# EleutherAI/DALLE-mtf

Hardware: AMD Instinct MI355X
Metric: train tokens/sec (text+image) per node, dalle_example (higher is better)
Workload: dtype bf16

## Files before the change

### dalle-mtf_amd/csrc/elementwise.hip

```cpp
#include "common.h"
#include <stdarg.h>

static thread_local char g_err[512] = "ok";
void dmi_set_error(const char* fmt, ...) {
  va_list ap;
  va_start(ap, fmt);
  vsnprintf(g_err, sizeof(g_err), fmt, ap);
  va_end(ap);
}
extern "C" const char* dmi_last_error_string(void) { return g_err; }
extern "C" int dmi_version(void) { return 100; }

__global__ __launch_bounds__(256) void embed_fwd_kernel(const int* __restrict__ tokens,
                                                        const bf16_t* __restrict__ wte,
                                                        const bf16_t* __restrict__ wpe, bf16_t* __restrict__ x,
                                                        int64_t rows, int S, int d, int vocab, const int* __restrict__ pos_dev) {
  const int lane = threadIdx.x & 63, wid = threadIdx.x >> 6;
  const int64_t row = (int64_t)blockIdx.x * 4 + wid;
  if (row >= rows) return;
  int tok = tokens[row];
  tok = tok < 0 ? 0 : (tok >= vocab ? vocab - 1 : tok);
  int s = (int)(row % S);
  if (pos_dev) {
    s = *pos_dev;
// ... 145 lines not shown
    float acc[8] = {0, 0, 0, 0, 0, 0, 0, 0};
    int cur = first_tok;
    bool open = head_open;
    bool first = true;
    for (int64_t i = i0; i < i1; ++i) {
      const int t = sorted_tok[i];
      if (t != cur) {
        float* dst = open ? part + ((int64_t)chunk * 2 + 0) * d + c * 8 : dwte + (int64_t)eb_clamp(cur, vocab) * d + c * 8;
        *(f32x4*)dst = f32x4{acc[0], acc[1], acc[2], acc[3]};
        *(f32x4*)(dst + 4) = f32x4{acc[4], acc[5], acc[6], acc[7]};
#pragma unroll
        for (int j = 0; j < 8; ++j) acc[j] = 0.f;
        cur = t;
        open = false;
        first = false;
      }
      float f[8];
      unpack8(*(const u32x4*)(dx + (int64_t)perm[i] * d + c * 8), f);
#pragma unroll
      for (int j = 0; j < 8; ++j) acc[j] += f[j];
    }
    const bool tail_open = (i1 < n) && (sorted_tok[i1] == cur);
    float* dst;
    if (open || tail_open) dst = part + ((int64_t)chunk * 2 + (first ? 0 : 1)) * d + c * 8;
    else dst = dwte + (int64_t)eb_clamp(cur, vocab) * d + c * 8;
    *(f32x4*)dst = f32x4{acc[0], acc[1], acc[2], acc[3]};
    *(f32x4*)(dst + 4) = f32x4{acc[4], acc[5], acc[6], acc[7]};
  }
}
__global__ __launch_bounds__(256) void embed_bwd_wte_combine_kernel(const int* __restrict__ sorted_tok, float* __restrict__ dwte,
                                                                    const float* __restrict__ part, int64_t n, int d, int vocab) {
  const int lane = threadIdx.x & 63, wid = threadIdx.x >> 6;
  const int64_t chunk = (int64_t)blockIdx.x * 4 + wid;
  const int64_t i0 = chunk * EB_CH;
  if (i0 >= n) return;
  const int64_t i1 = (i0 + EB_CH < n) ? i0 + EB_CH : n;
  if (i1 >= n) return;
  const int tok = sorted_tok[i1 - 1];
  if (sorted_tok[i1] != tok) return;
  const bool single = sorted_tok[i0] == tok;
  if (single && i0 > 0 && sorted_tok[i0 - 1] == tok) return;
  const int slot = single ? 0 : 1;
  const int64_t nchunks = (n + EB_CH - 1) / EB_CH;
  int64_t cnt = 0;
  for (int64_t base = chunk + 1; base < nchunks; base += 64) {
    const int64_t k = base + lane;
    bool cont = false, last = true;
    if (k < nchunks) {
      const int64_t k0 = k * EB_CH, k1 = (k0 + EB_CH < n) ? k0 + EB_CH : n;
      cont = sorted_tok[k0] == tok;
      last = !(sorted_tok[k1 - 1] == tok && k1 < n && sorted_tok[k1] == tok);
    }
    const unsigned long long stop = __ballot(!cont || last);
    if (stop == 0ull) { cnt += 64; continue; }
    const int f = __ffsll((long long)stop) - 1;
    const unsigned long long contb = __ballot(cont);
    cnt += f + (((contb >> f) & 1ull) ? 1 : 0);
    break;
  }
  const float* p0 = part + ((int64_t)chunk * 2 + slot) * d;
  const float* pk = part + ((int64_t)(chunk + 1) * 2) * d;
  for (int c = lane; c < d / 4; c += 64) {
    f32x4 acc = *(const f32x4*)(p0 + c * 4);
    int64_t k = 0;
    for (; k + 4 <= cnt; k += 4) {
      const f32x4 v0 = *(const f32x4*)(pk + (k + 0) * 2 * d + c * 4);
      const f32x4 v1 = *(const f32x4*)(pk + (k + 1) * 2 * d + c * 4);
      const f32x4 v2 = *(const f32x4*)(pk + (k + 2) * 2 * d + c * 4);
      const f32x4 v3 = *(const f32x4*)(pk + (k + 3) * 2 * d + c * 4);
#pragma unroll
      for (int j = 0; j < 4; ++j) acc[j] = (((acc[j] + v0[j]) + v1[j]) + v2[j]) + v3[j];
    }
    for (; k < cnt; ++k) {
      const f32x4 v = *(const f32x4*)(pk + k * 2 * d + c * 4);
      acc[0] += v[0]; acc[1] += v[1]; acc[2] += v[2]; acc[3] += v[3];
    }
    *(f32x4*)(dwte + (int64_t)eb_clamp(tok, vocab) * d + c * 4) = acc;
  }
}

extern "C" int64_t dmi_embed_bwd_workspace_bytes(int B, int S, int d) {
  return (((int64_t)B * S + EB_CH - 1) / EB_CH) * 2 * d * 4 + 256;
}
extern "C" int dmi_embed_bwd(const int32_t* sorted_tokens, const int32_t* perm, const uint16_t* dx, float* dwte,
                             float* dwpe, int B, int S, int d, int vocab, void* workspace, void* stream) {
  DMI_REQUIRE(sorted_tokens && perm && dx && dwte && dwpe && workspace, "embed_bwd: null pointer");
  DMI_REQUIRE(d % 8 == 0 && B > 0 && S > 0 && vocab > 0, "embed_bwd: bad sizes");
  hipStream_t st = (hipStream_t)stream;
  embed_bwd_wpe_kernel<<<dim3((S + 3) / 4), dim3(256), 0, st>>>(dx, dwpe, B, S, d);
  DMI_CHECK_LAUNCH("embed_bwd_wpe");
  DMI_REQUIRE(hipMemsetAsync(dwte, 0, (size_t)vocab * d * 4, st) == hipSuccess, "embed_bwd: memset failed");
  const int64_t n = (int64_t)B * S;
  const int64_t chunks = cdiv64(n, EB_CH);
  embed_bwd_wte_sorted_kernel<<<dim3((unsigned)cdiv64(chunks, 4)), dim3(256), 0, st>>>(sorted_tokens, perm, dx, dwte, (float*)workspace, n, d, vocab);
  DMI_CHECK_LAUNCH("embed_bwd_wte_sorted");
  embed_bwd_wte_combine_kernel<<<dim3((unsigned)cdiv64(chunks, 4)), dim3(256), 0, st>>>(sorted_tokens, dwte, (const float*)workspace, n, d, vocab);
  DMI_CHECK_LAUNCH("embed_bwd_wte_combine");
  return DMI_OK;
}

template <int NC>
__global__ __launch_bounds__(256) void ln_fwd_kernel(const bf16_t* __restrict__ x, const bf16_t* __restrict__ g,
                                                     const bf16_t* __restrict__ b, bf16_t* __restrict__ y,
                                                     float* __restrict__ mean, float* __restrict__ rstd,
                                                     int64_t rows, int d, float eps) {
  const int lane = threadIdx.x & 63, wid = threadIdx.x >> 6;
  const int64_t row = (int64_t)blockIdx.x * 4 + wid;
  if (row >= rows) return;
  const int nch = d / 8;
  float v[NC][8];
  float sum = 0.f;
#pragma unroll
  for (int i = 0; i < NC; ++i) {
    const int c = lane + 64 * i;
    if (c < nch) {
      unpack8(*(const u32x4*)(x + row * d + c * 8), v[i]);
#pragma unroll
      for (int j = 0; j < 8; ++j) sum += v[i][j];
    }
  }
  const float mu = wave_sum(sum) / (float)d;
  float sq = 0.f;
#pragma unroll
  for (int i = 0; i < NC; ++i) {
    const int c = lane + 64 * i;
    if (c < nch) {
#pragma unroll
      for (int j = 0; j < 8; ++j) {
        v[i][j] -= mu;
        sq += v[i][j] * v[i][j];
      }
    }
  }
  const float rs = rsqrtf(wave_sum(sq) / (float)d + eps);
#pragma unroll
  for (int i = 0; i < NC; ++i) {
    const int c = lane + 64 * i;
    if (c < nch) {
      float fg[8], fb[8], o[8];
      unpack8(*(const u32x4*)(g + c * 8), fg);
      unpack8(*(const u32x4*)(b + c * 8), fb);
#pragma unroll
      for (int j = 0; j < 8; ++j) o[j] = v[i][j] * rs * fg[j] + fb[j];
      *(u32x4*)(y + row * d + c * 8) = pack8(o);
    }
  }
  if (lane == 0) {
    mean[row] = mu;
    rstd[row] = rs;
  }
}

extern "C" int dmi_layernorm_fwd(const uint16_t* x, const uint16_t* g, const uint16_t* b, uint16_t* y, float* mean,
                                 float* rstd, int64_t rows, int d, float eps, void* stream) {
  DMI_REQUIRE(x && g && b && y && mean && rstd, "layernorm_fwd: null pointer");
  DMI_REQUIRE(d % 8 == 0 && d <= 4096 && rows > 0, "layernorm_fwd: unsupported d=%d (need d%%8==0, d<=4096)", d);
  hipStream_t st = (hipStream_t)stream;
  dim3 grid((unsigned)cdiv64(rows, 4)), blk(256);
  if (d <= 512) ln_fwd_kernel<1><<<grid, blk, 0, st>>>(x, g, b, y, mean, rstd, rows, d, eps);
  else if (d <= 1024) ln_fwd_kernel<2><<<grid, blk, 0, st>>>(x, g, b, y, mean, rstd, rows, d, eps);
  else if (d <= 2048) ln_fwd_kernel<4><<<grid, blk, 0, st>>>(x, g, b, y, mean, rstd, rows, d, eps);
  else ln_fwd_kernel<8><<<grid, blk, 0, st>>>(x, g, b, y, mean, rstd, rows, d, eps);
  DMI_CHECK_LAUNCH("layernorm_fwd");
  return DMI_OK;
}

__global__ __launch_bounds__(256) void reduce_partials_kernel(const float* __restrict__ part, float* __restrict__ out,
                                                              int P, int ncols) {
  __shared__ float sm[4][64];
  const int cl = threadIdx.x & 63, grp = threadIdx.x >> 6;
  const int c = blockIdx.x * 64 + cl;
  float acc = 0.f;
  if (c < ncols) {
    float a0 = 0.f, a1 = 0.f, a2 = 0.f, a3 = 0.f;
    int p = grp;
    for (; p + 12 < P; p += 16) {
      a0 += part[(int64_t)p * ncols + c];
      a1 += part[(int64_t)(p + 4) * ncols + c];
      a2 += part[(int64_t)(p + 8) * ncols + c];
      a3 += part[(int64_t)(p + 12) * ncols + c];
    }
    for (; p < P; p += 4) a0 += part[(int64_t)p * ncols + c];
    acc = (a0 + a1) + (a2 + a3);
  }
  sm[grp][cl] = acc;
  __syncthreads();
  if (grp == 0 && c < ncols) out[c] = (sm[0][cl] + sm[1][cl]) + (sm[2][cl] + sm[3][cl]);
}

#define LN_BWD_RPB 32
extern "C" int64_t dmi_layernorm_bwd_workspace_bytes(int64_t rows, int d) {
  return cdiv64(rows, LN_BWD_RPB) * 2 * (int64_t)d * 4;
}

template <int NC>
__global__ __launch_bounds__(256) void ln_bwd_kernel(const bf16_t* __restrict__ dy, const bf16_t* __restrict__ x,
                                                     const bf16_t* __restrict__ g, const float* __restrict__ mean,
                                                     const float* __restrict__ rstd, const bf16_t* __restrict__ dres,
                                                     bf16_t* __restrict__ dx, float* __restrict__ part,
                                                     int64_t rows, int d) {
  extern __shared__ __attribute__((aligned(16))) float sm[];
  const int lane = threadIdx.x & 63, wid = threadIdx.x >> 6;
  const int nch = d / 8;
  float ag[NC][8], ab[NC][8], fg[NC][8];
#pragma unroll
  for (int i = 0; i < NC; ++i) {
    const int c = lane + 64 * i;
#pragma unroll
    for (int j = 0; j < 8; ++j) ag[i][j] = ab[i][j] = 0.f;
    if (c < nch) unpack8(*(const u32x4*)(g + c * 8), fg[i]);
  }
  const int64_t r0 = (int64_t)blockIdx.x * LN_BWD_RPB;
  u32x4 rdy[NC], rx[NC], rr[NC];
  float mu_n = 0.f, rs_n = 0.f;
  auto fetch = [&](int64_t row) {
    if (row < rows) {
      mu_n = mean[row];
      rs_n = rstd[row];
#pragma unroll
      for (int i = 0; i < NC; ++i) {
        const int c = lane + 64 * i;
        if (c < nch) {
          rdy[i] = *(const u32x4*)(dy + row * d + c * 8);
          rx[i] = *(const u32x4*)(x + row * d + c * 8);
          if (dres) rr[i] = *(const u32x4*)(dres + row * d + c * 8);
        }
      }
    }
  };
  fetch(r0 + wid);
  for (int it = 0; it < LN_BWD_RPB / 4; ++it) {
    const int64_t row = r0 + wid + 4 * it;
    if (row >= rows) break;
    const float mu = mu_n, rs = rs_n;
    float fy[NC][8], xh[NC][8], fr[NC][8];
    float s1 = 0.f, s2 = 0.f;
#pragma unroll
    for (int i = 0; i < NC; ++i) {
      const int c = lane + 64 * i;
      if (c < nch) {
        float fx[8];
        unpack8(rdy[i], fy[i]);
        unpack8(rx[i], fx);
        if (dres) unpack8(rr[i], fr[i]);
#pragma unroll
        for (int j = 0; j < 8; ++j) {
// ... 123 lines not shown
  float a0 = 0.f, a1 = 0.f, a2 = 0.f, a3 = 0.f, a4 = 0.f, a5 = 0.f, a6 = 0.f, a7 = 0.f;
  if (c < nc) {
    int p = grp;
    for (; p + 112 < P; p += 128) {
      const float* q = part + (int64_t)p * nc + c;
      a0 += q[0];
      a1 += q[16 * nc];
      a2 += q[32 * nc];
      a3 += q[48 * nc];
      a4 += q[64 * nc];
      a5 += q[80 * nc];
      a6 += q[96 * nc];
      a7 += q[112 * nc];
    }
    for (; p < P; p += 16) a0 += part[(int64_t)p * nc + c];
  }
  sm[grp][cl] = ((a0 + a1) + (a2 + a3)) + ((a4 + a5) + (a6 + a7));
  __syncthreads();
  if (grp == 0 && c < nc) {
    float s = 0.f;
#pragma unroll
    for (int q = 0; q < 16; ++q) s += sm[q][cl];
    if (c < d) b.dg[it][c] = s;
    else b.db[it][c - d] = s;
  }
}
extern "C" int dmi_layernorm_bwd_finish_batch(const void* const* workspaces, float* const* dgs, float* const* dbs, const int64_t* rows,
                                              int n, int d, void* stream) {
  DMI_REQUIRE(workspaces && dgs && dbs && rows && n >= 1 && n <= LN_FINISH_MAX, "layernorm_bwd_finish_batch: 1..%d items", LN_FINISH_MAX);
  DMI_REQUIRE(d % 8 == 0 && d <= 2048, "layernorm_bwd_finish_batch: unsupported d=%d", d);
  LnFinishBatch b;
  b.d = d;
  for (int i = 0; i < n; ++i) {
    DMI_REQUIRE(workspaces[i] && dgs[i] && dbs[i] && rows[i] > 0, "layernorm_bwd_finish_batch: null pointer in item %d", i);
    b.part[i] = (const float*)workspaces[i]; b.dg[i] = dgs[i]; b.db[i] = dbs[i];
    b.P[i] = (int)cdiv64(rows[i], LN_BWD_RPB);
  }
  ln_bwd_finish_batch_kernel<<<dim3((2 * d + 15) / 16, n), dim3(256), 0, (hipStream_t)stream>>>(b);
  DMI_CHECK_LAUNCH("layernorm_bwd_finish_batch");
  return DMI_OK;
}

#define COLSUM_RPB 256
extern "C" int64_t dmi_colsum_workspace_bytes(int64_t M, int N) { return cdiv64(M, COLSUM_RPB) * (int64_t)N * 4; }

__global__ __launch_bounds__(256) void colsum_kernel(const bf16_t* __restrict__ Y, int ldy, float* __restrict__ part,
                                                     int64_t M, int N) {
  __shared__ float sm[4][64][8];
  const int cl = threadIdx.x & 63, rl = threadIdx.x >> 6;
  const int cg = blockIdx.x * 64 + cl;
  const int64_t r0 = (int64_t)blockIdx.y * COLSUM_RPB;
  const int64_t r1 = (r0 + COLSUM_RPB < M) ? r0 + COLSUM_RPB : M;
  float acc[8] = {0, 0, 0, 0, 0, 0, 0, 0};
  if (cg * 8 < N) {
    for (int64_t r = r0 + rl; r < r1; r += 4) {
      float f[8];
      unpack8(*(const u32x4*)(Y + r * ldy + cg * 8), f);
#pragma unroll
      for (int j = 0; j < 8; ++j) acc[j] += f[j];
    }
  }
#pragma unroll
  for (int j = 0; j < 8; ++j) sm[rl][cl][j] = acc[j];
  __syncthreads();
  if (rl == 0 && cg * 8 < N) {
#pragma unroll
    for (int j = 0; j < 8; ++j)
      part[(int64_t)blockIdx.y * N + cg * 8 + j] = (sm[0][cl][j] + sm[1][cl][j]) + (sm[2][cl][j] + sm[3][cl][j]);
  }
}

extern "C" int dmi_colsum(const uint16_t* Y, int ldy, float* out, int64_t M, int N, void* workspace, void* stream) {
  DMI_REQUIRE(Y && out && workspace, "colsum: null pointer");
  DMI_REQUIRE(N % 8 == 0 && ldy % 8 == 0 && M > 0, "colsum: N,ldy must be multiples of 8");
  hipStream_t st = (hipStream_t)stream;
  const int P = (int)cdiv64(M, COLSUM_RPB);
  colsum_kernel<<<dim3((N / 8 + 63) / 64, P), dim3(256), 0, st>>>(Y, ldy, (float*)workspace, M, N);
  DMI_CHECK_LAUNCH("colsum");
  reduce_partials_kernel<<<dim3((N + 63) / 64), dim3(256), 0, st>>>((const float*)workspace, out, P, N);
  DMI_CHECK_LAUNCH("colsum_reduce");
  return DMI_OK;
}

__device__ __forceinline__ void transpose_tile(const bf16_t* __restrict__ src, bf16_t* __restrict__ dst, int Rv, int R,
                                               int C, int64_t sr, int r0, int c0, unsigned (*t)[33]) {
  const int tid = threadIdx.x;
  {
    const int chunk = tid & 7, rp = tid >> 3;
    const int ra = r0 + 2 * rp, c = c0 + 8 * chunk;
    u32x4 va = {0, 0, 0, 0}, vb = {0, 0, 0, 0};
    if (c < C) {
      if (ra < Rv) va = *(const u32x4*)(src + (int64_t)ra * sr + c);
      if (ra + 1 < Rv) vb = *(const u32x4*)(src + (int64_t)(ra + 1) * sr + c);
    }
#pragma unroll
    for (int j = 0; j < 8; ++j) {
      const unsigned lo = (va[j >> 1] >> ((j & 1) * 16)) & 0xffffu;
      const unsigned hi = (vb[j >> 1] >> ((j & 1) * 16)) & 0xffffu;
      t[8 * chunk + j][rp] = lo | (hi << 16);
    }
  }
  __syncthreads();
  {
    const int orow = tid >> 2, seg = tid & 3;
    const int c = c0 + orow, r = r0 + 16 * seg;
    if (c < C) {
#pragma unroll
      for (int q = 0; q < 2; ++q) {
        const int rr = r + 8 * q;
        if (rr < R) {
          u32x4 v;
#pragma unroll
          for (int i = 0; i < 4; ++i) v[i] = t[orow][8 * seg + 4 * q + i];
          *(u32x4*)(dst + (int64_t)c * R + rr) = v;
        }
      }
    }
  }
}

__global__ __launch_bounds__(256) void transpose_kernel(const bf16_t* __restrict__ in, bf16_t* __restrict__ out,
                                                        int nh, int Rv, int R, int C, int64_t sb, int64_t sh, int64_t sr) {
  __shared__ unsigned t[64][33];
  const int bh = blockIdx.z, b = bh / nh, h = bh % nh;
  transpose_tile(in + b * sb + h * sh, out + (int64_t)bh * C * R, Rv, R, C, sr, blockIdx.y * 64, blockIdx.x * 64, t);
}

__global__ __launch_bounds__(256) void transpose_batch_kernel(const bf16_t* __restrict__ in, bf16_t* __restrict__ out,
                                                              const int64_t* __restrict__ table, int n) {
  __shared__ unsigned t[64][33];
  const int64_t tile = blockIdx.x;
  int i = 0;
  while (i + 1 < n && table[(i + 1) * 5 + 4] <= tile) ++i;
  const int64_t in_off = table[i * 5], out_off = table[i * 5 + 1];
  const int R = (int)table[i * 5 + 2], C = (int)table[i * 5 + 3];
  const int local = (int)(tile - table[i * 5 + 4]);
  const int tc = (C + 63) / 64;
  transpose_tile(in + in_off, out + out_off, R, R, C, C, (local / tc) * 64, (local % tc) * 64, t);
}
extern "C" int dmi_transpose_bf16_batch(const uint16_t* in_base, uint16_t* out_base, const int64_t* table, int n,
                                        int64_t total_tiles, void* stream) {
  DMI_REQUIRE(in_base && out_base && table && n > 0 && total_tiles > 0, "transpose_batch: bad args");
  transpose_batch_kernel<<<dim3((unsigned)total_tiles), dim3(256), 0, (hipStream_t)stream>>>(in_base, out_base, table, n);
  DMI_CHECK_LAUNCH("transpose_batch");
  return DMI_OK;
}

static int dmi_transpose_padded(const uint16_t* in, uint16_t* out, int nb, int nh, int Rv, int Rp, int C,
                         int64_t in_b_stride, int64_t in_h_stride, int64_t in_r_stride, void* stream) {
  DMI_REQUIRE(in && out, "transpose: null pointer");
  DMI_REQUIRE(Rp % 8 == 0 && Rp >= Rv && C % 8 == 0 && in_r_stride % 8 == 0 && in_h_stride % 8 == 0 && in_b_stride % 8 == 0,
              "transpose: R, C and strides must be multiples of 8 (R=%d C=%d)", Rp, C);
  transpose_kernel<<<dim3((C + 63) / 64, (Rp + 63) / 64, nb * nh), dim3(256), 0, (hipStream_t)stream>>>(
      in, out, nh, Rv, Rp, C, in_b_stride, in_h_stride, in_r_stride);
  DMI_CHECK_LAUNCH("transpose");
  return DMI_OK;
}
extern "C" int dmi_transpose_bf16_padded(const uint16_t* in, uint16_t* out, int R_valid, int R_pitch, int C, void* stream) {
  return dmi_transpose_padded(in, out, 1, 1, R_valid, R_pitch, C, 0, 0, C, stream);
}
extern "C" int dmi_transpose_bf16(const uint16_t* in, uint16_t* out, int batch, int R, int C, void* stream) {
  return dmi_transpose_padded(in, out, batch, 1, R, R, C, (int64_t)R * C, 0, C, stream);
}

__global__ void shift_labels_kernel(const int* __restrict__ tokens, int* __restrict__ labels, int B, int S, int eos) {
  const int64_t i = (int64_t)blockIdx.x * blockDim.x + threadIdx.x;
  if (i >= (int64_t)B * S) return;
  const int s = (int)(i % S);
  labels[i] = (s == S - 1) ? eos : tokens[i + 1];
}
extern "C" int dmi_shift_labels(const int32_t* tokens, int32_t* labels, int B, int S, int eos, void* stream) {
  DMI_REQUIRE(tokens && labels && B > 0 && S > 0, "shift_labels: bad args");
  const int64_t n = (int64_t)B * S;
  shift_labels_kernel<<<dim3((unsigned)cdiv64(n, 256)), dim3(256), 0, (hipStream_t)stream>>>(tokens, labels, B, S, eos);
  DMI_CHECK_LAUNCH("shift_labels");
  return DMI_OK;
}

__global__ __launch_bounds__(256) void assemble_tokens_kernel(const int* __restrict__ text,
                                                              const float* __restrict__ logits, int* __restrict__ out,
                                                              int B, int T, int P, int C, int text_vocab) {
  const int lane = threadIdx.x & 63, wid = threadIdx.x >> 6;
  const int64_t idx = (int64_t)blockIdx.x * 4 + wid;
  const int S = T + P;
  if (idx >= (int64_t)B * S) return;
  const int b = (int)(idx / S), s = (int)(idx % S);
  if (s < T) {
    if (lane == 0) out[idx] = text[(int64_t)b * T + s];
    return;
  }
  const float* row = logits + ((int64_t)b * P + (s - T)) * C;
  float best = -INFINITY;
  int bi = 0x7fffffff;
  for (int c = lane; c < C; c += 64) {
    const float v = row[c];
    if (v > best || (v == best && c < bi)) {
      best = v;
      bi = c;
    }
  }
#pragma unroll
// ... 143 lines not shown
  __syncthreads();
  const float k = dz_scale / bs;
  const int lch = (label >= 0 && label < V) ? (label >> 3) : -1, lj = label & 7;
#pragma unroll
  for (int i = 0; i < NC; ++i) {
    const int c = tid + 1024 * i;
    if (c < nch) {
#pragma unroll
      for (int j = 0; j < 8; ++j) f[i][j] *= k;
      if (c == lch) {
        asm volatile("" ::: "memory");
#pragma unroll
        for (int j = 0; j < 8; ++j) f[i][j] -= (j == lj) ? dz_scale : 0.f;
      }
      *(u32x4*)(zr + c * 8) = pack8(f[i]);
    }
  }
}

extern "C" int dmi_cross_entropy(uint16_t* z, int ldz, const int32_t* labels, float* loss_rows, float* lse,
                                 int64_t M, int V, float dz_scale, void* stream) {
  DMI_REQUIRE(z && labels && loss_rows, "cross_entropy: null pointer");
  DMI_REQUIRE(ldz % 8 == 0 && ldz >= ((V + 7) / 8) * 8 && M > 0 && V > 0, "cross_entropy: ldz must be a multiple of 8 and >= round_up(V,8)");
  hipStream_t st = (hipStream_t)stream;
  const int nch = ldz / 8;
  if (nch > 2048 && nch <= 8 * 1024) {
    if (nch <= 4 * 1024) cross_entropy_reg_kernel<4><<<dim3((unsigned)M), dim3(1024), 0, st>>>(z, ldz, labels, loss_rows, lse, V, dz_scale);
    else if (nch <= 7 * 1024) cross_entropy_reg_kernel<7><<<dim3((unsigned)M), dim3(1024), 0, st>>>(z, ldz, labels, loss_rows, lse, V, dz_scale);
    else cross_entropy_reg_kernel<8><<<dim3((unsigned)M), dim3(1024), 0, st>>>(z, ldz, labels, loss_rows, lse, V, dz_scale);
  } else {
    cross_entropy_kernel<<<dim3((unsigned)M), dim3(256), 0, st>>>(z, ldz, labels, loss_rows, lse, V, dz_scale);
  }
  DMI_CHECK_LAUNCH("cross_entropy");
  return DMI_OK;
}

__global__ __launch_bounds__(256) void label_logit_kernel(const bf16_t* __restrict__ X, int ldx, const bf16_t* __restrict__ Wt,
                                                          int ldw, const bf16_t* __restrict__ bias, const int* __restrict__ labels,
                                                          float* __restrict__ zl, int* __restrict__ flag, int64_t M, int K, int V) {
  const int lane = threadIdx.x & 63, wid = threadIdx.x >> 6;
  if (blockIdx.x == 0 && threadIdx.x == 0) flag[0] = 0;
  const int64_t row = (int64_t)blockIdx.x * 4 + wid;
  if (row >= M) return;
  int lab = labels[row];
  lab = lab < 0 ? 0 : (lab >= V ? V - 1 : lab);
  const bf16_t* xr = X + row * ldx;
  const bf16_t* wr = Wt + (int64_t)lab * ldw;
  float acc = 0.f;
  for (int c = lane; c < K / 8; c += 64) {
    float a[8], b[8];
    unpack8(*(const u32x4*)(xr + c * 8), a);
    unpack8(*(const u32x4*)(wr + c * 8), b);
#pragma unroll
    for (int j = 0; j < 8; ++j) acc = __builtin_fmaf(a[j], b[j], acc);
  }
  acc = wave_sum(acc);
  if (lane == 0) zl[row] = acc + bf2f(bias[lab]);
}
extern "C" int dmi_label_logit(const uint16_t* X, int ldx, const uint16_t* Wt, int ldw, const uint16_t* bias,
                               const int32_t* labels, float* zl, int32_t* flag, int64_t M, int K, int V, void* stream) {
  DMI_REQUIRE(X && Wt && bias && labels && zl && flag, "label_logit: null pointer");
  DMI_REQUIRE(M > 0 && K % 8 == 0 && ldx % 8 == 0 && ldw % 8 == 0 && V > 0, "label_logit: bad sizes");
  label_logit_kernel<<<dim3((unsigned)cdiv64(M, 4)), dim3(256), 0, (hipStream_t)stream>>>(X, ldx, Wt, ldw, bias, labels, zl, flag, M, K, V);
  DMI_CHECK_LAUNCH("label_logit");
  return DMI_OK;
}

struct SoftmaxFinishArgs {
  const float* part; int nparts;
  const float* zl;
  const float* rowshift;
  const int* labels;
  const bf16_t* X; int ldx;
  bf16_t* E; int lde;
  float* loss_rows; float* rowscale; bf16_t* rowscale_bf16; bf16_t* Xs;
  int* flag;
  int64_t M; int K, V;
  float dz_scale;
};
#define SF_ROWS 64
#define SF_PARTS 16
struct NoWeight { static constexpr bool on = false; };
struct PosWeight { static constexpr bool on = true; const float* w; int period; };
template <class PW>
__global__ __launch_bounds__(256) void softmax_finish_kernel(SoftmaxFinishArgs a, PW pw) {
  __shared__ float sm[SF_PARTS][SF_ROWS];
  __shared__ float sc[SF_ROWS];
  const int tid = threadIdx.x, r4 = tid & 15, q = tid >> 4;
  const int64_t m0 = (int64_t)blockIdx.x * SF_ROWS, m = m0 + 4 * r4;
  f32x4 s = {0.f, 0.f, 0.f, 0.f};
  if (m + 3 < a.M && (a.M & 3) == 0) {
    for (int p = q; p < a.nparts; p += SF_PARTS) {
      const f32x4 v = *(const f32x4*)(a.part + (int64_t)p * a.M + m);
      s[0] += v[0]; s[1] += v[1]; s[2] += v[2]; s[3] += v[3];
    }
  } else {
    for (int j = 0; j < 4; ++j)
      if (m + j < a.M)
        for (int p = q; p < a.nparts; p += SF_PARTS) s[j] += a.part[(int64_t)p * a.M + m + j];
  }
#pragma unroll
  for (int j = 0; j < 4; ++j) sm[q][4 * r4 + j] = s[j];
  __syncthreads();
  if (tid < SF_ROWS) {
    const int r = tid;
    const int64_t mr = m0 + r;
    float scale = 0.f;
    if (mr < a.M) {
      float S = 0.f;
#pragma unroll
      for (int k = 0; k < SF_PARTS; ++k) S += sm[k][r];
      const bool bad = !(S > 1.0e-18f && S < 1.0e18f);
      if (bad) a.flag[0] = 1;
      a.loss_rows[mr] = bad ? INFINITY : __logf(S) + (a.rowshift ? a.rowshift[mr] : 0.f) - a.zl[mr];
      float dz = a.dz_scale;
      if constexpr (PW::on) dz *= pw.w[(int)(((int64_t)(m0 % pw.period) + r) % pw.period)];
      scale = bad ? 0.f : dz / S;
      if (a.dz_scale != 0.f) {
        a.rowscale[mr] = scale;
        a.rowscale_bf16[mr] = f2bf(scale);
        int lab = a.labels[mr];
        lab = lab < 0 ? 0 : (lab >= a.V ? a.V - 1 : lab);
        bf16_t* el = a.E + mr * a.lde + lab;
        *el = f2bf(bf2f(*el) - S);
      }
    }
    sc[r] = scale;
  }
  __syncthreads();
  if (a.dz_scale == 0.f) return;
  const int cpr = a.K / 8;
  for (int idx = tid; idx < SF_ROWS * cpr; idx += 256) {
    const int rr = idx / cpr, ch = idx - rr * cpr;
    const int64_t mm = m0 + rr;
    if (mm >= a.M) break;
    float f[8];
    unpack8(*(const u32x4*)(a.X + mm * a.ldx + ch * 8), f);
    const float k = sc[rr];
#pragma unroll
    for (int j = 0; j < 8; ++j) f[j] *= k;
    *(u32x4*)(a.Xs + mm * a.K + ch * 8) = pack8(f);
  }
}
#define FIX_MAXK 8192
template <class PW>
__global__ __launch_bounds__(256) void softmax_fixup_kernel(SoftmaxFinishArgs a, const bf16_t* __restrict__ Wt, int ldw,
                                                            const bf16_t* __restrict__ bias, int N, PW pw) {
  if (a.flag[0] == 0) return;
  __shared__ float xs[FIX_MAXK];
  __shared__ float red[4];
  __shared__ float zlab;
  const int tid = threadIdx.x, lane = tid & 63, wid = tid >> 6;
  for (int64_t m = blockIdx.x; m < a.M; m += gridDim.x) {
    if (a.loss_rows[m] < 3.0e38f) continue;
    __syncthreads();
    for (int k = tid; k < a.K; k += 256) xs[k] = bf2f(a.X[m * a.ldx + k]);
    int lab = a.labels[m];
    lab = lab < 0 ? 0 : (lab >= a.V ? a.V - 1 : lab);
    __syncthreads();
    auto logit = [&](int v) {
      const bf16_t* wr = Wt + (int64_t)v * ldw;
      float acc = 0.f;
      for (int c = lane; c < a.K / 8; c += 64) {
        float b[8];
        unpack8(*(const u32x4*)(wr + c * 8), b);
#pragma unroll
        for (int j = 0; j < 8; ++j) acc = __builtin_fmaf(xs[c * 8 + j], b[j], acc);
      }
      return wave_sum(acc) + bf2f(bias[v]);
    };
    float mx = -INFINITY;
    for (int v = wid; v < a.V; v += 4) {
      const float z = logit(v);
      mx = fmaxf(mx, z);
      if (v == lab && lane == 0) zlab = z;
    }
    if (lane == 0) red[wid] = mx;
    __syncthreads();
    mx = fmaxf(fmaxf(red[0], red[1]), fmaxf(red[2], red[3]));
    const float zl = zlab;
    __syncthreads();
    float sum = 0.f;
    for (int v = wid; v < N; v += 4) {
      const float e = (v < a.V) ? __expf(logit(v) - mx) : 0.f;
      sum += e;
      if (lane == 0) a.E[m * a.lde + v] = f2bf(e);
    }
    if (lane == 0) red[wid] = sum;
    __syncthreads();
    const float S = ((red[0] + red[1]) + red[2]) + red[3];
    float dz = a.dz_scale;
    if constexpr (PW::on) dz *= pw.w[(int)(m % pw.period)];
    const float scale = dz / S;
    __syncthreads();
    if (tid == 0) {
      a.loss_rows[m] = mx + __logf(S) - zl;
      if (a.dz_scale != 0.f) {
        a.rowscale[m] = scale;
        a.rowscale_bf16[m] = f2bf(scale);
        a.E[m * a.lde + lab] = f2bf(__expf(zl - mx) - S);
      }
    }
    if (a.dz_scale != 0.f)
      for (int k = tid * 8; k < a.K; k += 256 * 8) {
        float f[8];
#pragma unroll
        for (int j = 0; j < 8; ++j) f[j] = xs[k + j] * scale;
        *(u32x4*)(a.Xs + m * a.K + k) = pack8(f);
      }
  }
}
static int softmax_finish_launch(const float* rowsum_part, int nparts, const float* label_logit, const float* rowshift,
                                 const int32_t* labels, const uint16_t* X, int ldx,
                                 const uint16_t* Wt, int ldw, const uint16_t* bias, uint16_t* E, int lde, int N,
                                 float* loss_rows, float* rowscale, uint16_t* rowscale_bf16, uint16_t* Xs, int32_t* flag,
                                 int64_t M, int K, int V, float dz_scale, const float* pos_weight, int period, void* stream) {
  DMI_REQUIRE(rowsum_part && label_logit && labels && X && Wt && bias && E && loss_rows && flag, "softmax_finish: null pointer");
  DMI_REQUIRE(dz_scale == 0.f || (rowscale && rowscale_bf16 && Xs), "softmax_finish: gradient outputs missing");
  DMI_REQUIRE(M > 0 && K % 8 == 0 && K <= FIX_MAXK && ldx % 8 == 0 && ldw % 8 == 0 && nparts > 0 && V > 0 && V <= N && N <= lde,
              "softmax_finish: bad sizes (K <= %d)", FIX_MAXK);
  SoftmaxFinishArgs a;
  a.part = rowsum_part; a.nparts = nparts; a.zl = label_logit; a.rowshift = rowshift; a.labels = labels; a.X = X; a.ldx = ldx; a.E = E; a.lde = lde;
  a.loss_rows = loss_rows; a.rowscale = rowscale; a.rowscale_bf16 = rowscale_bf16; a.Xs = Xs; a.flag = flag;
  a.M = M; a.K = K; a.V = V; a.dz_scale = dz_scale;
  hipStream_t st = (hipStream_t)stream;
  const PosWeight pw{pos_weight, period};
  if (pos_weight) softmax_finish_kernel<<<dim3((unsigned)cdiv64(M, SF_ROWS)), dim3(256), 0, st>>>(a, pw);
  else softmax_finish_kernel<<<dim3((unsigned)cdiv64(M, SF_ROWS)), dim3(256), 0, st>>>(a, NoWeight{});
  DMI_CHECK_LAUNCH("softmax_finish");
  if (pos_weight) softmax_fixup_kernel<<<dim3(256), dim3(256), 0, st>>>(a, Wt, ldw, bias, N, pw);
  else softmax_fixup_kernel<<<dim3(256), dim3(256), 0, st>>>(a, Wt, ldw, bias, N, NoWeight{});
  DMI_CHECK_LAUNCH("softmax_fixup");
  return DMI_OK;
}
extern "C" int dmi_softmax_finish(const float* rowsum_part, int nparts, const float* label_logit, const float* rowshift,
                                  const int32_t* labels, const uint16_t* X, int ldx,
                                  const uint16_t* Wt, int ldw, const uint16_t* bias, uint16_t* E, int lde, int N,
                                  float* loss_rows, float* rowscale, uint16_t* rowscale_bf16, uint16_t* Xs, int32_t* flag,
                                  int64_t M, int K, int V, float dz_scale, void* stream) {
  return softmax_finish_launch(rowsum_part, nparts, label_logit, rowshift, labels, X, ldx, Wt, ldw, bias, E, lde, N, loss_rows, rowscale,
                               rowscale_bf16, Xs, flag, M, K, V, dz_scale, nullptr, 0, stream);
}
extern "C" int dmi_softmax_finish_w(const float* rowsum_part, int nparts, const float* label_logit, const float* rowshift,
                                    const int32_t* labels, const uint16_t* X, int ldx,
                                    const uint16_t* Wt, int ldw, const uint16_t* bias, uint16_t* E, int lde, int N,
                                    float* loss_rows, float* rowscale, uint16_t* rowscale_bf16, uint16_t* Xs, int32_t* flag,
                                    int64_t M, int K, int V, float dz_scale, const float* pos_weight, int period, void* stream) {
  DMI_REQUIRE(pos_weight, "softmax_finish_w: null pos_weight");
  DMI_REQUIRE(period > 0, "softmax_finish_w: period must be > 0");
  return softmax_finish_launch(rowsum_part, nparts, label_logit, rowshift, labels, X, ldx, Wt, ldw, bias, E, lde, N, loss_rows, rowscale,
                               rowscale_bf16, Xs, flag, M, K, V, dz_scale, pos_weight, period, stream);
}

__device__ __forceinline__ float block_sum_256(float x, float* sm) {
  x = wave_sum(x);
  if ((threadIdx.x & 63) == 0) sm[threadIdx.x >> 6] = x;
  __syncthreads();
  return (sm[0] + sm[1]) + (sm[2] + sm[3]);
}

__global__ __launch_bounds__(1024) void sum_f32_kernel(const float* __restrict__ x, int64_t n, float scale,
                                                       float* __restrict__ out) {
  __shared__ float sm[16];
  const int tid = threadIdx.x;
  float a0 = 0.f, a1 = 0.f, a2 = 0.f, a3 = 0.f;
  if ((((uintptr_t)x) & 15) == 0) {
    const int64_t n4 = n / 4;
    const f32x4* x4 = (const f32x4*)x;
    int64_t i = tid;
    for (; i + 3072 < n4; i += 4096) {
      const f32x4 v0 = x4[i], v1 = x4[i + 1024], v2 = x4[i + 2048], v3 = x4[i + 3072];
      a0 += (v0[0] + v0[1]) + (v0[2] + v0[3]);
      a1 += (v1[0] + v1[1]) + (v1[2] + v1[3]);
      a2 += (v2[0] + v2[1]) + (v2[2] + v2[3]);
      a3 += (v3[0] + v3[1]) + (v3[2] + v3[3]);
    }
    for (; i < n4; i += 1024) {
      const f32x4 v0 = x4[i];
      a0 += (v0[0] + v0[1]) + (v0[2] + v0[3]);
    }
    if (tid < (n & 3)) a1 += x[n4 * 4 + tid];
  } else {
    for (int64_t i = tid; i < n; i += 1024) a0 += x[i];
  }
  float t = wave_sum((a0 + a1) + (a2 + a3));
  if ((tid & 63) == 0) sm[tid >> 6] = t;
  __syncthreads();
  if (tid == 0) {
    float r = 0.f;
#pragma unroll
    for (int w = 0; w < 16; ++w) r += sm[w];
    out[0] = r * scale;
  }
}
extern "C" int dmi_sum_f32(const float* x, int64_t n, float scale, float* out, void* stream) {
  DMI_REQUIRE(x && out && n > 0, "sum_f32: bad args");
  sum_f32_kernel<<<dim3(1), dim3(1024), 0, (hipStream_t)stream>>>(x, n, scale, out);
  DMI_CHECK_LAUNCH("sum_f32");
  return DMI_OK;
}

__global__ __launch_bounds__(1024) void loss_reduce_kernel(const float* __restrict__ loss_rows, int64_t M,
                                                           const float* __restrict__ pos_weight, int period, int split,
                                                           float scale, float inv_text, float inv_image, float* __restrict__ out3) {
  __shared__ float sm[3][16];
  const int tid = threadIdx.x;
  const int step = 1024 % period;
  int pos = tid % period;
  float aw = 0.f, at = 0.f, ai = 0.f;
  for (int64_t m = tid; m < M; m += 1024) {
    const float l = loss_rows[m];
    aw = __builtin_fmaf(pos_weight[pos], l, aw);
    if (pos < split) at += l; else ai += l;
    pos += step;
    if (pos >= period) pos -= period;
  }
  aw = wave_sum(aw); at = wave_sum(at); ai = wave_sum(ai);
  if ((tid & 63) == 0) { sm[0][tid >> 6] = aw; sm[1][tid >> 6] = at; sm[2][tid >> 6] = ai; }
  __syncthreads();
  if (tid < 3) {
    const float* s = sm[tid];
    const float r = (((s[0] + s[1]) + (s[2] + s[3])) + ((s[4] + s[5]) + (s[6] + s[7]))) +
                    (((s[8] + s[9]) + (s[10] + s[11])) + ((s[12] + s[13]) + (s[14] + s[15])));
    out3[tid] = r * (tid == 0 ? scale : tid == 1 ? inv_text : inv_image);
  }
}
extern "C" int dmi_loss_reduce(const float* loss_rows, int64_t M, const float* pos_weight, int period, int split, float scale,
                               float* out3, void* stream) {
  DMI_REQUIRE(loss_rows && pos_weight && out3, "loss_reduce: null pointer");
  DMI_REQUIRE(M > 0 && period > 0 && split >= 0 && split <= period, "loss_reduce: bad sizes (M > 0, period > 0, 0 <= split <= period)");
  const int64_t full = M / period, rem = M % period;
  const int64_t ntext = full * split + (rem < split ? rem : split), nimage = M - ntext;
  loss_reduce_kernel<<<dim3(1), dim3(1024), 0, (hipStream_t)stream>>>(loss_rows, M, pos_weight, period, split, scale,
                                                                      ntext ? (float)(1.0 / (double)ntext) : 0.f,
                                                                      nimage ? (float)(1.0 / (double)nimage) : 0.f, out3);
  DMI_CHECK_LAUNCH("loss_reduce");
  return DMI_OK;
}

#define SUMSQ_BLOCKS 2048
extern "C" int64_t dmi_sumsq_workspace_bytes(int64_t n) { (void)n; return SUMSQ_BLOCKS * 4; }
__global__ __launch_bounds__(256) void sumsq_kernel(const float* __restrict__ g, int64_t n, float* __restrict__ part) {
  __shared__ float sm[4];
  float acc = 0.f;
  const int64_t n4 = n / 4;
  const f32x4* g4 = (const f32x4*)g;
  for (int64_t i = (int64_t)blockIdx.x * 256 + threadIdx.x; i < n4; i += (int64_t)gridDim.x * 256) {
    const f32x4 v = g4[i];
    acc += (v[0] * v[0] + v[1] * v[1]) + (v[2] * v[2] + v[3] * v[3]);
  }
  if (blockIdx.x == 0 && threadIdx.x < (n & 3)) {
    const float v = g[n4 * 4 + threadIdx.x];
    acc += v * v;
  }
  const float t = block_sum_256(acc, sm);
  if (threadIdx.x == 0) part[blockIdx.x] = t;
}
extern "C" int dmi_sumsq(const float* g, int64_t n, float* out, void* workspace, void* stream) {
  DMI_REQUIRE(g && out && workspace && n > 0, "sumsq: bad args");
  DMI_REQUIRE(((uintptr_t)g & 15) == 0, "sumsq: g must be 16-byte aligned");
  hipStream_t st = (hipStream_t)stream;
  sumsq_kernel<<<dim3(SUMSQ_BLOCKS), dim3(256), 0, st>>>(g, n, (float*)workspace);
  DMI_CHECK_LAUNCH("sumsq");
  sum_f32_kernel<<<dim3(1), dim3(1024), 0, st>>>((const float*)workspace, SUMSQ_BLOCKS, 1.0f, out);
  DMI_CHECK_LAUNCH("sumsq_finish");
  return DMI_OK;
}

__global__ __launch_bounds__(256) void adam_kernel(float* __restrict__ p, const float* __restrict__ g,
                                                   float* __restrict__ m, float* __restrict__ v,
                                                   bf16_t* __restrict__ pb, int64_t n,
                                                   const float* __restrict__ gnorm_sq, float clip, float lr, float b1,
                                                   float b2, float eps, float wd, float gscale,
                                                   const float* __restrict__ lr_dev) {
  if (lr_dev) lr = lr_dev[0];
  float mult = gscale;
  if (gnorm_sq != nullptr && clip > 0.f) {
    const float gn = sqrtf(gnorm_sq[0]) * gscale;
    mult = gscale * (clip / fmaxf(gn, clip));
  }
  const int64_t n4 = n / 4;
  for (int64_t i = (int64_t)blockIdx.x * 256 + threadIdx.x; i < n4; i += (int64_t)gridDim.x * 256) {
    f32x4 pv = ((f32x4*)p)[i], gv = ((const f32x4*)g)[i], mv = ((f32x4*)m)[i], vv = ((f32x4*)v)[i];
#pragma unroll
    for (int j = 0; j < 4; ++j) {
      const float gg = gv[j] * mult;
      mv[j] = b1 * mv[j] + (1.f - b1) * gg;
      vv[j] = b2 * vv[j] + (1.f - b2) * gg * gg;
      float upd = mv[j] / (sqrtf(vv[j]) + eps);
      upd += wd * pv[j];
      pv[j] -= lr * upd;
    }
    ((f32x4*)p)[i] = pv;
    ((f32x4*)m)[i] = mv;
    ((f32x4*)v)[i] = vv;
    if (pb) *(u32x2*)(pb + i * 4) = u32x2{pack2bf(pv[0], pv[1]), pack2bf(pv[2], pv[3])};
  }
  if (blockIdx.x == 0 && threadIdx.x < (n & 3)) {
    const int64_t i = n4 * 4 + threadIdx.x;
    const float gg = g[i] * mult;
    const float mm = b1 * m[i] + (1.f - b1) * gg;
    const float vv = b2 * v[i] + (1.f - b2) * gg * gg;
    float pp = p[i];
    pp -= lr * (mm / (sqrtf(vv) + eps) + wd * pp);
    p[i] = pp;
    m[i] = mm;
    v[i] = vv;
    if (pb) pb[i] = f2bf(pp);
  }
}
extern "C" int dmi_adam_step(float* p, const float* g, float* m, float* v, uint16_t* p_bf16, int64_t n,
                             const float* gnorm_sq, float clip, float lr, float beta1, float beta2, float eps,
                             float weight_decay, float grad_scale, const float* lr_dev, void* stream) {
  DMI_REQUIRE(p && g && m && v && n > 0, "adam_step: bad args");
  DMI_REQUIRE((((uintptr_t)p | (uintptr_t)g | (uintptr_t)m | (uintptr_t)v) & 15) == 0 && (((uintptr_t)p_bf16) & 7) == 0,
              "adam_step: buffers must be 16-byte aligned");
  int64_t blocks = cdiv64(n / 4 + 1, 256);
  if (blocks > 4096) blocks = 4096;
  adam_kernel<<<dim3((unsigned)blocks), dim3(256), 0, (hipStream_t)stream>>>(p, g, m, v, p_bf16, n, gnorm_sq, clip, lr, beta1, beta2, eps, weight_decay, grad_scale, lr_dev);
  DMI_CHECK_LAUNCH("adam_step");
  return DMI_OK;
}

__global__ __launch_bounds__(256) void cast_kernel(const float* __restrict__ in, bf16_t* __restrict__ out, int64_t n) {
  for (int64_t i = (int64_t)blockIdx.x * 256 + threadIdx.x; i < n; i += (int64_t)gridDim.x * 256) out[i] = f2bf(in[i]);
}
extern "C" int dmi_cast_f32_bf16(const float* in, uint16_t* out, int64_t n, void* stream) {
  DMI_REQUIRE(in && out && n > 0, "cast: bad args");
  int64_t blocks = cdiv64(n, 256);
  if (blocks > 8192) blocks = 8192;
  cast_kernel<<<dim3((unsigned)blocks), dim3(256), 0, (hipStream_t)stream>>>(in, out, n);
  DMI_CHECK_LAUNCH("cast");
  return DMI_OK;
}

__device__ __forceinline__ unsigned order_key(float v) {
  const unsigned u = __float_as_uint(v);
  return (u & 0x80000000u) ? ~u : (u | 0x80000000u);
}
__device__ __forceinline__ float key_value(unsigned k) { return __uint_as_float((k & 0x80000000u) ? (k & 0x7fffffffu) : ~k); }
__device__ __forceinline__ uint64_t splitmix64(uint64_t x) {
  x += 0x9E3779B97F4A7C15ull;
  x = (x ^ (x >> 30)) * 0xBF58476D1CE4E5B9ull;
  x = (x ^ (x >> 27)) * 0x94D049BB133111EBull;
  return x ^ (x >> 31);
}
#define SAMPLE_MAX_VOCAB 8192
__global__ __launch_bounds__(256) void sample_tokens_kernel(const bf16_t* __restrict__ z, int ldz, const bf16_t* __restrict__ bias, int nv,
                                                            float inv_temp, int top_k, uint64_t seed, const unsigned* __restrict__ params_dev,
                                                            int pos_arg, int* pos_dev, int advance, int token_offset,
                                                            int* __restrict__ next_tok, int* __restrict__ out, int out_ld, int out_col0) {
  __shared__ unsigned keys[SAMPLE_MAX_VOCAB];
  __shared__ int cnt[4];
  __shared__ float bval[4];
  __shared__ int bidx[4];
  const int b = blockIdx.x, tid = threadIdx.x, lane = tid & 63, wid = tid >> 6;
  if (params_dev) {
    inv_temp = __uint_as_float(params_dev[0]);
    top_k = (int)params_dev[1];
    seed = (uint64_t)params_dev[2] | ((uint64_t)params_dev[3] << 32);
  }
  const int counter = pos_dev ? *pos_dev : pos_arg;
  const bool greedy = !(inv_temp > 0.f);
  for (int i = tid; i < nv; i += 256) {
    float v = bf2f(z[(int64_t)b * ldz + i]);
    if (bias) v += bf2f(bias[i]);
    if (!greedy) v *= inv_temp;
    keys[i] = order_key(v);
  }
  __syncthreads();
  unsigned thr = 0u;
  if (!greedy && top_k > 0 && top_k < nv) {
    for (int bit = 31; bit >= 0; --bit) {
      const unsigned cand = thr | (1u << bit);
      int c = 0;
      for (int i = tid; i < nv; i += 256) c += keys[i] >= cand;
#pragma unroll
      for (int o = 32; o > 0; o >>= 1) c += __shfl_xor(c, o, 64);
      if (lane == 0) cnt[wid] = c;
      __syncthreads();
      const int total = cnt[0] + cnt[1] + cnt[2] + cnt[3];
      __syncthreads();
      if (total >= top_k) thr = cand;
    }
  }
  const uint64_t stream_key = splitmix64(seed ^ ((uint64_t)(unsigned)counter * 0xD2B74407B1CE6E93ull));
  float best = -INFINITY;
  int besti = nv;
  for (int i = tid; i < nv; i += 256) {
    const unsigned k = keys[i];
    if (k < thr) continue;
    float s = key_value(k);
    if (!greedy) {
      const uint64_t h = splitmix64(stream_key + (((uint64_t)(unsigned)b << 32) | (unsigned)i));
      const float u = ((float)(unsigned)(h >> 41) + 0.5f) * (1.0f / 8388608.0f);
      s -= __logf(-__logf(u));
    }
    if (s > best) { best = s; besti = i; }
  }
#pragma unroll
  for (int o = 32; o > 0; o >>= 1) {
    const float ob = __shfl_xor(best, o, 64);
    const int oi = __shfl_xor(besti, o, 64);
// ... 285 lines not shown
```

### dalle-mtf_amd/dalle_hip/__init__.py

```python
from __future__ import annotations

import ctypes
import os
import re
import struct

import numpy as np
from ctypes import c_char_p, c_float, c_int, c_int64, c_void_p

import torch

_HERE = os.path.dirname(os.path.abspath(__file__))
LIB_PATH = os.environ.get("DALLE_HIP_LIB") or os.path.join(_HERE, "libdalle_hip.so")
HEADER_PATH = os.path.join(os.path.dirname(os.path.dirname(_HERE)), "include", "dalle_hip.h")

GEMM_BIAS, GEMM_RELU, GEMM_RESIDUAL, GEMM_RELU_MASK, GEMM_OUT_F32, GEMM_ROWSCALE = 1, 2, 4, 8, 16, 32
GEMM_GELU = 512

_lib = None


class DalleHipError(RuntimeError):
    pass


def declared_symbols():
    txt = open(HEADER_PATH).read()
    return sorted(set(re.findall(r"\b(dmi_[a-z0-9_]+)\s*\(", txt)))


def lib():
    global _lib
    if _lib is None:
        if not os.path.exists(LIB_PATH):
            raise DalleHipError(
                f"{LIB_PATH} not found: build it with `python __graft_entry__.py` (hipcc --offload-arch=gfx950). "
                "There is no CPU fallback for the product path.")
        _lib = ctypes.CDLL(LIB_PATH)
        _declare(_lib)
        for kv in os.environ.get("DALLE_HIP_OPTIONS", "").split(","):
            if "=" in kv:
                if _lib.dmi_set_option(kv.split("=")[0].strip().encode(), int(kv.split("=")[1])) != 0:
                    raise DalleHipError(f"DALLE_HIP_OPTIONS: unknown option {kv!r}")
    return _lib


def _declare(L):
    P, I, L64, F = c_void_p, c_int, c_int64, c_float
    sig = {
        "dmi_last_error_string": (c_char_p, []),
        "dmi_version": (I, []),
        "dmi_get_option": (I, [c_char_p]),
        "dmi_set_option": (I, [c_char_p, I]),
        "dmi_set_debug_buffer": (I, [P]),
        "dmi_embed_fwd": (I, [P, P, P, P, L64, I, I, I, P, P]),
        "dmi_sort_tokens_workspace_bytes": (L64, [L64]),
        "dmi_sort_tokens": (I, [P, P, P, L64, I, P, P]),
        "dmi_embed_bwd_workspace_bytes": (L64, [I, I, I]),
        "dmi_embed_bwd": (I, [P, P, P, P, P, I, I, I, I, P, P]),
        "dmi_layernorm_fwd": (I, [P, P, P, P, P, P, L64, I, F, P]),
        "dmi_layernorm_bwd_workspace_bytes": (L64, [L64, I]),
        "dmi_layernorm_bwd": (I, [P, P, P, P, P, P, P, P, P, P, L64, I, P]),
        "dmi_layernorm_bwd_finish_batch": (I, [P, P, P, P, I, I, P]),
        "dmi_gemm_nt": (I, [P, I, P, I, P, I, I, I, I, I, P, P, P, P, P]),
        "dmi_gemm_nt_splitk_workspace_bytes": (L64, [I, I, I]),
        "dmi_gemm_nt_splitk": (I, [P, I, P, I, P, I, I, I, I, P, P, P]),
        "dmi_gemm_tn_workspace_bytes": (L64, [I, I, I]),
        "dmi_gemm_tn": (I, [P, I, P, I, P, P, P, I, I, I, P, P, P, P]),
        "dmi_gemm_tn_group": (I, [P, I, I, P, P, P]),
        "dmi_gemm_tn_group_plan": (I, [P, P, I, I]),
        "dmi_reduce_slabs_batch": (I, [P, I, P]),
        "dmi_colsum_workspace_bytes": (L64, [L64, I]),
        "dmi_colsum": (I, [P, I, P, L64, I, P, P]),
        "dmi_transpose_bf16": (I, [P, P, I, I, I, P]),
        "dmi_attention_fwd": (I, [P, P, P, I, I, I, P]),
        "dmi_attention_bwd": (I, [P, P, P, P, P, P, I, I, I, P]),
        "dmi_attention_decode": (I, [P, P, P, I, I, I, I, P, P]),
        "dmi_attention_fwd_hd": (I, [P, P, P, I, I, I, I, P]),
        "dmi_attention_bwd_hd": (I, [P, P, P, P, P, P, I, I, I, I, P]),
        "dmi_attention_decode_hd": (I, [P, P, P, I, I, I, I, P, I, P]),
        "dmi_attn_mask_plan": (L64, [P, I, P, L64]),
        "dmi_attention_fwd_masked": (I, [P, P, P, P, P, I, I, I, I, P]),
        "dmi_attention_bwd_masked": (I, [P, P, P, P, P, P, P, P, I, I, I, I, P]),
        "dmi_attention_decode_masked": (I, [P, P, P, P, P, I, I, I, I, P, I, P]),
        "dmi_label_logit": (I, [P, I, P, I, P, P, P, P, L64, I, I, P]),
        "dmi_gemm_nt_softmax_partials": (L64, [I]),
        "dmi_gemm_nt_softmax": (I, [P, I, P, I, P, P, P, I, P, I, I, I, P]),
        "dmi_softmax_finish": (I, [P, I, P, P, P, P, I, P, I, P, P, I, I, P, P, P, P, P, L64, I, I, F, P]),
        "dmi_softmax_finish_w": (I, [P, I, P, P, P, P, I, P, I, P, P, I, I, P, P, P, P, P, L64, I, I, F, P, I, P]),
        "dmi_loss_reduce": (I, [P, L64, P, I, I, F, P, P]),
        "dmi_shift_labels": (I, [P, P, I, I, I, P]),
        "dmi_cross_entropy": (I, [P, I, P, P, P, L64, I, F, P]),
        "dmi_sum_f32": (I, [P, L64, F, P, P]),
        "dmi_assemble_tokens": (I, [P, P, P, I, I, I, I, I, P]),
        "dmi_sample_tokens": (I, [P, I, P, I, I, F, I, ctypes.c_uint64, P, I, P, I, I, P, P, I, I, P]),
        "dmi_sample_tokens_p": (I, [P, I, P, I, I, F, I, ctypes.c_uint64, F, P, I, P, I, I, P, P, I, I, P, P]),
        "dmi_sample_tokens_guided": (I, [P, I, P, I, I, F, I, ctypes.c_uint64, F, F, P, I, P, I, I, P, P, I, I, P, P]),
        "dmi_ln_gemm_nt": (I, [P, I, P, P, F, P, I, P, I, I, I, I, I, P, P]),
        "dmi_logits_f32": (I, [P, I, P, P, I, I, P]),
        "dmi_gemm_nt_ln": (I, [P, I, P, I, P, I, I, I, I, P, P, P, P, F, P, I, P, P, P]),
        "dmi_gemm_nt_lnbwd_parts": (I, [I]),
        "dmi_gemm_nt_lnbwd": (I, [P, I, P, I, I, I, I, P, P, P, P, P, P, P, P, I, P, P]),
        "dmi_layernorm_bwd_finish_parts": (I, [P, I, P, P, I, P]),
        "dmi_relu_bits_bytes": (L64, [I, I]),
        "dmi_relu_bits_auto": (I, [I, I, I]),
        "dmi_gemm_nt_ln_auto": (I, [I, I, I]),
        "dmi_gemm_nt_relu_bits": (I, [P, I, P, I, P, I, I, I, I, P, P, P]),
        "dmi_gemm_nt_mask_bits": (I, [P, I, P, I, P, I, I, I, I, P, P]),
        "dmi_gemm_nt_gelu": (I, [P, I, P, I, P, I, I, I, I, P, P, I, P]),
        "dmi_gemm_nt_gelu_grad": (I, [P, I, P, I, P, I, I, I, I, P, I, P]),
        "dmi_sumsq_workspace_bytes": (L64, [L64]),
        "dmi_sumsq": (I, [P, L64, P, P, P]),
        "dmi_adam_step": (I, [P, P, P, P, P, L64, P, F, F, F, F, F, F, F, P, P]),
        "dmi_adafactor_plan": (I, [P, I, P]),
        "dmi_adafactor_step": (I, [P, I, P, P, P, P, P, P, P, F, F, P, F, F, F, F, P, L64, P]),
        "dmi_cast_f32_bf16": (I, [P, P, L64, P]),
        "dmi_transpose_bf16_padded": (I, [P, P, I, I, I, P]),
        "dmi_transpose_bf16_batch": (I, [P, P, P, I, L64, P]),
        "dmi_im2col": (I, [P, P, I, I, I, I, I, I, I, I, P, P, I, P]),
        "dmi_conv_gemm_nt": (I, [P, I, I, I, I, I, I, I, I, P, P, P, I, P, I, I, I, P, P, P, P]),
        "dmi_conv_wgrad_tn_workspace_bytes": (L64, [I, I, I]),
        "dmi_conv_wgrad_tn": (I, [P, I, I, I, I, I, I, I, I, P, P, P, I, I, P, P, P, P, P, P]),
        "dmi_weight_gather": (I, [P, P, I, I, I, P, I, P]),
        "dmi_weight_gather_batch": (I, [P, P, P, I, L64, P]),
        "dmi_pixel_interleave": (I, [P, P, I, I, I, I, P]),
        "dmi_pad_channels": (I, [P, P, L64, I, I, P]),
        "dmi_unpad_channels": (I, [P, P, L64, I, I, P]),
        "dmi_gumbel_softmax_fwd": (I, [P, P, P, P, P, L64, I, F, I, P, P]),
        "dmi_gumbel_softmax_bwd": (I, [P, P, P, L64, I, F, P, P]),
        "dmi_mse_workspace_bytes": (L64, []),
        "dmi_mse_loss": (I, [P, P, P, P, L64, I, I, F, P, P]),
        "dmi_add_f32": (I, [P, P, L64, P]),
        "dmi_comm_load": (I, [c_char_p]),
        "dmi_comm_unique_id_bytes": (I, []),
        "dmi_comm_unique_id": (I, [P]),
        "dmi_comm_init": (I, [P, I, I, P]),
        "dmi_comm_destroy": (I, [P]),
        "dmi_allreduce_bucket": (I, [P, P, L64, P]),
        "dmi_comm_broadcast_f32": (I, [P, P, L64, I, P]),
        "dmi_conv2d_f32": (I, [P, I, I, I, I, I, I, I, I, P, P, P, P, P, P, I, I, P]),
        "dmi_space_to_depth_f32": (I, [P, P, I, I, I, I, I, I, P]),
        "dmi_depth_to_space_f32": (I, [P, P, I, I, I, I, I, I, P]),
        "dmi_crc32c": (ctypes.c_uint32, [c_char_p, ctypes.c_size_t]),
    }
    for name, (res, args) in sig.items():
        fn = getattr(L, name)
        fn.restype = res
        fn.argtypes = args


def _check(rc, what):
    if rc != 0:
        raise DalleHipError(f"{what}: status {rc}: {lib().dmi_last_error_string().decode()}")


def _p(t):
    if t is None:
        return 0
    return t if isinstance(t, int) else t.data_ptr()


def _stream():
    return torch.cuda.current_stream().cuda_stream


def _dev(*ts):
    for t in ts:
        if t is not None and not isinstance(t, int) and not t.is_cuda:
            raise DalleHipError("dalle_hip ops need CUDA(HIP) tensors; there is no CPU fallback")


def set_option(name: str, value: int):
    _check(lib().dmi_set_option(name.encode(), int(value)), "set_option")


def get_option(name: str) -> int:
    return lib().dmi_get_option(name.encode())



def embed_fwd(tokens, wte, wpe, x, S, d, vocab, pos_dev=None):
    _dev(tokens, wte, wpe, x)
    _check(lib().dmi_embed_fwd(_p(tokens), _p(wte), _p(wpe), _p(x), tokens.numel(), S, d, vocab, _p(pos_dev), _stream()), "embed_fwd")


def sort_tokens_workspace_bytes(n):
    return int(lib().dmi_sort_tokens_workspace_bytes(n))


def sort_tokens(tokens, sorted_tokens, perm, n, vocab, ws):
    _dev(tokens, sorted_tokens, perm, ws)
    _check(lib().dmi_sort_tokens(_p(tokens), _p(sorted_tokens), _p(perm), n, vocab, _p(ws), _stream()), "sort_tokens")


def embed_bwd_workspace_bytes(B, S, d):
    return int(lib().dmi_embed_bwd_workspace_bytes(B, S, d))


def embed_bwd(sorted_tokens, perm, dx, dwte, dwpe, B, S, d, vocab, ws):
    _dev(sorted_tokens, perm, dx, dwte, dwpe, ws)
    _check(lib().dmi_embed_bwd(_p(sorted_tokens), _p(perm), _p(dx), _p(dwte), _p(dwpe), B, S, d, vocab, _p(ws), _stream()),
           "embed_bwd")


def layernorm_fwd(x, g, b, y, mean, rstd, rows, d, eps=1e-5):
    _dev(x, g, b, y, mean, rstd)
    _check(lib().dmi_layernorm_fwd(_p(x), _p(g), _p(b), _p(y), _p(mean), _p(rstd), rows, d, eps, _stream()), "layernorm_fwd")


def layernorm_bwd_workspace_bytes(rows, d):
    return lib().dmi_layernorm_bwd_workspace_bytes(rows, d)


def layernorm_bwd(dy, x, g, mean, rstd, dres, dx, dg, db, ws, rows, d):
    _dev(dy, x, g, mean, rstd, dx, ws)
    _check(lib().dmi_layernorm_bwd(_p(dy), _p(x), _p(g), _p(mean), _p(rstd), _p(dres), _p(dx), _p(dg), _p(db),
                                   _p(ws), rows, d, _stream()), "layernorm_bwd")


def layernorm_bwd_finish_batch(items, d):
    import ctypes
    n = len(items)
    PA, LA = ctypes.c_void_p * n, ctypes.c_int64 * n
    _check(lib().dmi_layernorm_bwd_finish_batch(PA(*[_p(i[0]) for i in items]), PA(*[_p(i[1]) for i in items]), PA(*[_p(i[2]) for i in items]),
                                                LA(*[int(i[3]) for i in items]), n, d, _stream()), "layernorm_bwd_finish_batch")


def gemm_nt(A, lda, Bt, ldb, C, ldc, M, N, K, flags=0, bias=None, residual=None, relu_src=None, rowscale=None):
    _dev(A, Bt, C)
    _check(lib().dmi_gemm_nt(_p(A), lda, _p(Bt), ldb, _p(C), ldc, M, N, K, flags, _p(bias), _p(residual),
                             _p(relu_src), _p(rowscale), _stream()), "gemm_nt")


def gemm_nt_ln(A, lda, Bt, ldb, C, ldc, M, N, K, gamma, beta, Y, ldy, mean, rstd, bias=None, residual=None, eps=1e-5):
    _dev(A, Bt, C, gamma, beta, Y, mean, rstd)
    assert mean.dtype == torch.float32 and rstd.dtype == torch.float32 and mean.numel() >= M and rstd.numel() >= M
    _check(lib().dmi_gemm_nt_ln(_p(A), lda, _p(Bt), ldb, _p(C), ldc, M, N, K, _p(bias), _p(residual), _p(gamma), _p(beta), float(eps),
                                _p(Y), ldy, _p(mean), _p(rstd), _stream()), "gemm_nt_ln")


def gemm_nt_lnbwd_parts(M):
    return int(lib().dmi_gemm_nt_lnbwd_parts(M))


def gemm_nt_lnbwd(A, lda, Bt, ldb, M, N, K, x, gamma, mean, rstd, dres, dx, part, dg=None, db=None, B2=None, ldb2=0, C2=None):
    _dev(A, Bt, x, gamma, mean, rstd, dres, dx, part, dg, db, B2, C2)
    P = gemm_nt_lnbwd_parts(M)
    assert part.dtype == torch.float32 and part.numel() >= P * 2 * N
    _check(lib().dmi_gemm_nt_lnbwd(_p(A), lda, _p(Bt), ldb, M, N, K, _p(x), _p(gamma), _p(mean), _p(rstd), _p(dres), _p(dx), _p(part),
                                   _p(B2), ldb2, _p(C2), _stream()), "gemm_nt_lnbwd")
    if dg is not None:
        _check(lib().dmi_layernorm_bwd_finish_parts(_p(part), P, _p(dg), _p(db), N, _stream()), "layernorm_bwd_finish_parts")


def relu_bits_bytes(M, N):
    return int(lib().dmi_relu_bits_bytes(M, N))


def gemm_nt_ln_auto(M, N, K):
    return bool(lib().dmi_gemm_nt_ln_auto(M, N, K))


def relu_bits_auto(M, N, K):
    return bool(lib().dmi_relu_bits_auto(M, N, K))


def gemm_nt_relu_bits(A, lda, Bt, ldb, C, ldc, M, N, K, bias, bits):
    _dev(A, Bt, C, bias, bits)
    assert bits.dtype == torch.uint8 and bits.numel() >= relu_bits_bytes(M, N)
    _check(lib().dmi_gemm_nt_relu_bits(_p(A), lda, _p(Bt), ldb, _p(C), ldc, M, N, K, _p(bias), _p(bits), _stream()), "gemm_nt_relu_bits")


def gemm_nt_mask_bits(A, lda, Bt, ldb, C, ldc, M, N, K, bits):
    _dev(A, Bt, C, bits)
    assert bits.dtype == torch.uint8 and bits.numel() >= relu_bits_bytes(M, N)
    _check(lib().dmi_gemm_nt_mask_bits(_p(A), lda, _p(Bt), ldb, _p(C), ldc, M, N, K, _p(bits), _stream()), "gemm_nt_mask_bits")


def gemm_nt_gelu(A, lda, Bt, ldb, C, ldc, M, N, K, bias, pre, ldpre):
    _dev(A, Bt, C, bias, pre)
    _check(lib().dmi_gemm_nt_gelu(_p(A), lda, _p(Bt), ldb, _p(C), ldc, M, N, K, _p(bias), _p(pre), ldpre, _stream()), "gemm_nt_gelu")


def gemm_nt_gelu_grad(A, lda, Bt, ldb, C, ldc, M, N, K, pre, ldpre):
    _dev(A, Bt, C, pre)
# ... 129 lines not shown
PLAN_MAGIC = 0x504D4144
PLAN_HDR = dict(S=1, NB=2, W=3, CAUSAL=4, FPTR=5, FLIST=6, KPTR=7, KLIST=8, FORDER=9, KORDER=10, ROWBITS=11, COLBITS=12, WORDS=13,
                LIVE_F=14, CAUSAL_F=15, LIVE_K=16, CAUSAL_K=17)


class AttnMaskPlan:

    def __init__(self, mask, device="cuda"):
        m = np.ascontiguousarray(np.asarray(mask.cpu() if hasattr(mask, "cpu") else mask).astype(np.uint8))
        if m.ndim != 2 or m.shape[0] != m.shape[1]:
            raise DalleHipError(f"attn_mask_plan: the mask must be [S, S] (got {m.shape})")
        self.S = int(m.shape[0])
        fn = lib().dmi_attn_mask_plan
        nbytes = fn(m.ctypes.data, self.S, None, 0)
        if nbytes < 0:
            _check(int(nbytes), "attn_mask_plan")
        self.host = np.zeros(nbytes // 4, dtype=np.int32)
        _check(0 if fn(m.ctypes.data, self.S, self.host.ctypes.data, nbytes) == nbytes else -1, "attn_mask_plan")
        assert self.host[0] == PLAN_MAGIC and self.host[PLAN_HDR["S"]] == self.S
        self.causal = bool(self.host[PLAN_HDR["CAUSAL"]])
        self.dev = torch.from_numpy(self.host).to(device) if device is not None else None

    def live_fraction(self):
        return float(self.host[PLAN_HDR["LIVE_F"]]) / float(self.host[PLAN_HDR["CAUSAL_F"]])

    def live_fraction_dkv(self):
        return float(self.host[PLAN_HDR["LIVE_K"]]) / float(self.host[PLAN_HDR["CAUSAL_K"]])


def attn_mask_plan_bytes(mask_u8, S):
    m = np.ascontiguousarray(mask_u8, dtype=np.uint8)
    return int(lib().dmi_attn_mask_plan(m.ctypes.data, int(S), None, 0))


def attention_fwd_masked(qkv, o, lse, plan, B, H, S, head_dim=128):
    _dev(qkv, o, lse)
    _check(lib().dmi_attention_fwd_masked(_p(qkv), _p(o), _p(lse), _p(plan.dev), plan.host.ctypes.data, B, H, S, int(head_dim),
                                          _stream()), "attention_fwd_masked")


def attention_bwd_masked(qkv, o, d_o, lse, scratch, dqkv, plan, B, H, S, head_dim=128):
    _dev(qkv, o, d_o, lse, scratch, dqkv)
    _check(lib().dmi_attention_bwd_masked(_p(qkv), _p(o), _p(d_o), _p(lse), _p(scratch), _p(dqkv), _p(plan.dev), plan.host.ctypes.data,
                                          B, H, S, int(head_dim), _stream()), "attention_bwd_masked")


def attention_decode_masked(qkv, o, plan, B, H, S, pos, fresh=None, pos_dev=None, head_dim=128):
    _check(lib().dmi_attention_decode_masked(_p(qkv), _p(fresh), _p(o), _p(plan.dev), plan.host.ctypes.data, B, H, S, int(pos),
                                             _p(pos_dev), int(head_dim), _stream()), "attention_decode_masked")


def shift_labels(tokens, labels, B, S, eos):
    _dev(tokens, labels)
    _check(lib().dmi_shift_labels(_p(tokens), _p(labels), B, S, eos, _stream()), "shift_labels")


def cross_entropy(z, ldz, labels, loss_rows, lse, M, V, dz_scale):
    _dev(z, labels, loss_rows)
    _check(lib().dmi_cross_entropy(_p(z), ldz, _p(labels), _p(loss_rows), _p(lse), M, V, dz_scale, _stream()), "cross_entropy")


def label_logit(X, ldx, Wt, ldw, bias, labels, zl, flag, M, K, V):
    _dev(X, Wt, bias, labels, zl, flag)
    _check(lib().dmi_label_logit(_p(X), ldx, _p(Wt), ldw, _p(bias), _p(labels), _p(zl), _p(flag), M, K, V, _stream()), "label_logit")


def gemm_nt_softmax_partials(N):
    return int(lib().dmi_gemm_nt_softmax_partials(N))


def gemm_nt_softmax(X, ldx, Wt, ldw, bias, rowshift, E, lde, rowsum_part, M, N, K):
    _dev(X, Wt, bias, E, rowsum_part)
    _check(lib().dmi_gemm_nt_softmax(_p(X), ldx, _p(Wt), ldw, _p(bias), _p(rowshift), _p(E), lde, _p(rowsum_part), M, N, K,
                                     _stream()), "gemm_nt_softmax")


def softmax_finish(rowsum_part, nparts, label_logit, rowshift, labels, X, ldx, Wt, ldw, bias, E, lde, N, loss_rows, rowscale,
                   rowscale_bf16, Xs, flag, M, K, V, dz_scale):
    _dev(rowsum_part, label_logit, rowshift, labels, X, Wt, bias, E, loss_rows, flag)
    _check(lib().dmi_softmax_finish(_p(rowsum_part), nparts, _p(label_logit), _p(rowshift), _p(labels), _p(X), ldx, _p(Wt), ldw,
                                    _p(bias), _p(E), lde, N,
                                    _p(loss_rows), _p(rowscale), _p(rowscale_bf16), _p(Xs), _p(flag), M, K, V, float(dz_scale),
                                    _stream()), "softmax_finish")


def softmax_finish_w(rowsum_part, nparts, label_logit, rowshift, labels, X, ldx, Wt, ldw, bias, E, lde, N, loss_rows, rowscale,
                     rowscale_bf16, Xs, flag, M, K, V, dz_scale, pos_weight, period):
    _dev(rowsum_part, label_logit, rowshift, labels, X, Wt, bias, E, loss_rows, flag, pos_weight)
    _check(lib().dmi_softmax_finish_w(_p(rowsum_part), nparts, _p(label_logit), _p(rowshift), _p(labels), _p(X), ldx, _p(Wt), ldw,
                                      _p(bias), _p(E), lde, N,
                                      _p(loss_rows), _p(rowscale), _p(rowscale_bf16), _p(Xs), _p(flag), M, K, V, float(dz_scale),
                                      _p(pos_weight), int(period), _stream()), "softmax_finish_w")


def sum_f32(x, n, scale, out):
    _dev(x, out)
    _check(lib().dmi_sum_f32(_p(x), n, scale, _p(out), _stream()), "sum_f32")


def loss_reduce(loss_rows, n, pos_weight, period, split, scale, out3):
    _dev(loss_rows, pos_weight, out3)
    _check(lib().dmi_loss_reduce(_p(loss_rows), n, _p(pos_weight), int(period), int(split), float(scale), _p(out3), _stream()),
           "loss_reduce")


def assemble_tokens(text, vae_logits, tokens_out, B, T, P, C, text_vocab):
    _dev(text, vae_logits, tokens_out)
    _check(lib().dmi_assemble_tokens(_p(text), _p(vae_logits), _p(tokens_out), B, T, P, C, text_vocab, _stream()), "assemble_tokens")


def sample_tokens(z, ldz, bias, B, nv, temperature=1.0, top_k=0, seed=0, pos=0, token_offset=0, next_tok=None, out=None,
                  out_col0=0, params_dev=None, pos_dev=None, advance=False):
    _dev(z)
    assert z.dtype == torch.bfloat16 and (bias is None or bias.dtype == torch.bfloat16)
    if pos_dev is not None:
        assert pos_dev.dtype == torch.int32 and pos_dev.numel() >= (2 if advance else 1), \
            "sample_tokens: pos_dev must be int32 [2] ([position, zeroed counter]) when advance=True, int32 [1] otherwise"
    for t in (bias, next_tok, out, params_dev, pos_dev):
        if t is not None:
            _dev(t)
    out_ld = int(out.shape[1]) if out is not None else 0
    _check(lib().dmi_sample_tokens(_p(z), ldz, _p(bias), B, nv, float(temperature), int(top_k), int(seed) & (2 ** 64 - 1),
                                   _p(params_dev), int(pos), _p(pos_dev), int(bool(advance)), int(token_offset), _p(next_tok), _p(out), out_ld,
                                   int(out_col0), _stream()), "sample_tokens")


def sample_tokens_p(z, ldz, bias, B, nv, temperature=1.0, top_k=0, seed=0, top_p=1.0, pos=0, token_offset=0, next_tok=None,
                    out=None, out_col0=0, params_dev=None, pos_dev=None, advance=False, logp=None):
    _dev(z)
    assert z.dtype == torch.bfloat16 and (bias is None or bias.dtype == torch.bfloat16)
    if pos_dev is not None:
        assert pos_dev.dtype == torch.int32 and pos_dev.numel() >= (2 if advance else 1), \
            "sample_tokens_p: pos_dev must be int32 [2] ([position, zeroed counter]) when advance=True, int32 [1] otherwise"
    if params_dev is not None:
        assert params_dev.numel() >= 6 and params_dev.element_size() == 4, "sample_tokens_p: params_dev must be 32-bit [6]"
    if logp is not None:
        assert logp.dtype == torch.float32 and logp.numel() >= B, "sample_tokens_p: logp must be fp32 [B]"
    for t in (bias, next_tok, out, params_dev, pos_dev, logp):
        if t is not None:
            _dev(t)
    out_ld = int(out.shape[1]) if out is not None else 0
    _check(lib().dmi_sample_tokens_p(_p(z), ldz, _p(bias), B, nv, float(temperature), int(top_k), int(seed) & (2 ** 64 - 1),
                                     float(top_p), _p(params_dev), int(pos), _p(pos_dev), int(bool(advance)), int(token_offset),
                                     _p(next_tok), _p(out), out_ld, int(out_col0), _p(logp), _stream()), "sample_tokens_p")


def sample_tokens_guided(z, ldz, bias, Bc, nv, temperature=1.0, top_k=0, seed=0, top_p=1.0, scale=1.0, pos=0, token_offset=0,
                         next_tok=None, out=None, out_col0=0, params_dev=None, pos_dev=None, advance=False, logp=None):
    _dev(z)
    assert z.dtype == torch.bfloat16 and (bias is None or bias.dtype == torch.bfloat16)
    if pos_dev is not None:
        assert pos_dev.dtype == torch.int32 and pos_dev.numel() >= (2 if advance else 1), \
            "sample_tokens_guided: pos_dev must be int32 [2] ([position, zeroed counter]) when advance=True, int32 [1] otherwise"
    if params_dev is not None:
        assert params_dev.numel() >= 6 and params_dev.element_size() == 4, "sample_tokens_guided: params_dev must be 32-bit [6]"
    if next_tok is not None:
        assert next_tok.dtype == torch.int32 and next_tok.numel() >= 2 * Bc, "sample_tokens_guided: next_tok must be int32 [2 * Bc]"
    if out is not None:
        assert out.dtype == torch.int32 and out.dim() == 2 and out.shape[0] >= Bc, "sample_tokens_guided: out must be int32 [Bc, n]"
    if logp is not None:
        assert logp.dtype == torch.float32 and logp.numel() >= Bc, "sample_tokens_guided: logp must be fp32 [Bc]"
    for t in (bias, next_tok, out, params_dev, pos_dev, logp):
        if t is not None:
            _dev(t)
    out_ld = int(out.shape[1]) if out is not None else 0
    _check(lib().dmi_sample_tokens_guided(_p(z), ldz, _p(bias), Bc, nv, float(temperature), int(top_k), int(seed) & (2 ** 64 - 1),
                                          float(top_p), float(scale), _p(params_dev), int(pos), _p(pos_dev), int(bool(advance)),
                                          int(token_offset), _p(next_tok), _p(out), out_ld, int(out_col0), _p(logp), _stream()),
           "sample_tokens_guided")


def sample_params(temperature=1.0, top_k=0, seed=0, top_p=None, guidance_scale=None):
    def bits(x):
        return struct.unpack("<I", struct.pack("<f", x))[0]
    words = [bits(1.0 / temperature if temperature > 0 else 0.0), int(top_k), int(seed) & 0xffffffff, (int(seed) >> 32) & 0xffffffff]
    if guidance_scale is not None:
        assert top_p is not None, "sample_params: guidance_scale goes with top_p (the six-word block)"
        words += [bits(top_p), bits(guidance_scale)]
    elif top_p is not None:
        words += [bits(top_p), 0]
    return torch.tensor([w - (1 << 32) if w >= (1 << 31) else w for w in words], dtype=torch.int32)


def logits_f32(z, ldz, bias, out, B, nv):
    _dev(z, out)
    assert z.dtype == torch.bfloat16 and out.dtype == torch.float32 and out.is_contiguous() and out.numel() >= B * nv
    if bias is not None:
        _dev(bias)
        assert bias.dtype == torch.bfloat16
    _check(lib().dmi_logits_f32(_p(z), int(ldz), _p(bias), _p(out), int(B), int(nv), _stream()), "logits_f32")


def sumsq_workspace_bytes(n):
    return lib().dmi_sumsq_workspace_bytes(n)


def sumsq(g, n, out, ws):
    _dev(g, out, ws)
    _check(lib().dmi_sumsq(_p(g), n, _p(out), _p(ws), _stream()), "sumsq")


def adam_step(p, g, m, v, p_bf16, n, gnorm_sq, clip, lr, beta1, beta2, eps, wd, grad_scale=1.0, lr_dev=None):
    _dev(p, g, m, v)
    _check(lib().dmi_adam_step(_p(p), _p(g), _p(m), _p(v), _p(p_bf16), n, _p(gnorm_sq), clip, lr, beta1, beta2, eps,
                               wd, grad_scale, _p(lr_dev), _stream()), "adam_step")


AF_FIELDS = 17


def adafactor_plan(table):
    assert table.dtype == torch.int64 and not table.is_cuda and table.is_contiguous() and table.shape[1] == AF_FIELDS
    totals = torch.zeros(3, dtype=torch.int64)
    _check(lib().dmi_adafactor_plan(_p(table), table.shape[0], _p(totals)), "adafactor_plan")
    return tuple(int(x) for x in totals)


def adafactor_step(table_dev, nvars, totals, p, g, m, slots, p_bf16, gnorm_sq, clip, lr, decay, beta1, eps1, eps2, ws,
                   lr_dev=None):
    _dev(table_dev, p, g, m, slots, gnorm_sq, ws)
    tot = (ctypes.c_int64 * 3)(*totals)
    _check(lib().dmi_adafactor_step(_p(table_dev), nvars, ctypes.addressof(tot), _p(p), _p(g), _p(m), _p(slots), _p(p_bf16),
                                    _p(gnorm_sq), clip, lr, _p(lr_dev), decay, beta1, eps1, eps2, _p(ws), ws.numel() * ws.element_size(),
                                    _stream()), "adafactor_step")


def cast_f32_bf16(inp, out, n):
    _dev(inp, out)
    _check(lib().dmi_cast_f32_bf16(_p(inp), _p(out), n, _stream()), "cast_f32_bf16")



def transpose_padded(inp, out, R_valid, R_pitch, C):
    _dev(inp, out)
    _check(lib().dmi_transpose_bf16_padded(_p(inp), _p(out), R_valid, R_pitch, C, _stream()), "transpose_padded")


def _iarr(vals):
    return (ctypes.c_int * len(vals))(*[int(v) for v in vals])


def conv_gemm_nt(x, B, H, W, C, Ho, Wo, stride, taps, Wt, ldw, out, ldc, N, flags=0, bias=None, residual=None, relu_src=None):
    _dev(x, Wt, out)
    dy, dx = _iarr([t[0] for t in taps]), _iarr([t[1] for t in taps])
    _check(lib().dmi_conv_gemm_nt(_p(x), B, H, W, C, Ho, Wo, stride, len(taps), ctypes.cast(dy, c_void_p),
                                  ctypes.cast(dx, c_void_p), _p(Wt), ldw, _p(out), ldc, N, flags,
                                  _p(bias), _p(residual), _p(relu_src), _stream()), "conv_gemm_nt")


def conv_wgrad_tn_workspace_bytes(M, K, N):
    return int(lib().dmi_conv_wgrad_tn_workspace_bytes(M, K, N))


def conv_wgrad_tn(x, B, H, W, C, Ho, Wo, stride, taps, dY, ldy, N, dW, ws, dbias=None, deferred: "DeferredReduces" = None):
    _dev(x, dY, dW, ws)
    dy, dx = _iarr([t[0] for t in taps]), _iarr([t[1] for t in taps])
    if deferred is None:
        _check(lib().dmi_conv_wgrad_tn(_p(x), B, H, W, C, Ho, Wo, stride, len(taps), ctypes.cast(dy, c_void_p),
                                       ctypes.cast(dx, c_void_p), _p(dY), ldy, N, _p(dW), _p(dbias), _p(ws), None, None, _stream()),
               "conv_wgrad_tn")
        return
    assert deferred.n + 2 <= deferred.capacity
    cnt = c_int(0)
    slot = ctypes.byref(deferred.items, deferred.n * ctypes.sizeof(ReduceItem))
    _check(lib().dmi_conv_wgrad_tn(_p(x), B, H, W, C, Ho, Wo, stride, len(taps), ctypes.cast(dy, c_void_p),
                                   ctypes.cast(dx, c_void_p), _p(dY), ldy, N, _p(dW), _p(dbias), _p(ws), slot, ctypes.byref(cnt),
                                   _stream()), "conv_wgrad_tn")
    deferred.n += cnt.value


def im2col(x, out, B, H, W, C, Ho, Wo, stride, taps, ldo):
    _dev(x, out)
    dy, dx = _iarr([t[0] for t in taps]), _iarr([t[1] for t in taps])
    _check(lib().dmi_im2col(_p(x), _p(out), B, H, W, C, Ho, Wo, stride, len(taps), ctypes.cast(dy, c_void_p),
                            ctypes.cast(dx, c_void_p), ldo, _stream()), "im2col")


def weight_gather(inp, out, A, Bn, idx, ldo):
    _dev(inp, out)
    ia = _iarr(idx)
    _check(lib().dmi_weight_gather(_p(inp), _p(out), A, Bn, len(idx), ctypes.cast(ia, c_void_p), ldo, _stream()), "weight_gather")


def pixel_interleave(in4, out, B, Ht, Wt, C):
    _dev(in4, out)
    _check(lib().dmi_pixel_interleave(_p(in4), _p(out), B, Ht, Wt, C, _stream()), "pixel_interleave")


def pad_channels(inp, out, N, Cin, Cp):
    _dev(inp, out)
# ... 92 lines not shown
```

### dalle-mtf_amd/src/dalle_mtf/engine.py

```python
from __future__ import annotations

import contextlib
import gc
import hashlib
import math
import os
from collections import OrderedDict
from typing import Dict, List, Optional, Tuple

import numpy as np
import torch

import dalle_hip as dh
from ..dp import GradReducer
from .activations import check_activation
from .loss_weights import position_weights, resolve_loss_weights

@contextlib.contextmanager
def _no_gc_in_capture():
    gc.collect()
    was_enabled = gc.isenabled()
    gc.disable()
    try:
        yield
# ... 208 lines not shown
                out[r["name"] + "_slot_vr"], out[r["name"] + "_slot_vc"] = (vrow, vcol) if r["vr_row"] else (vcol, vrow)
            else:
                out[r["name"] + "_slot_v"] = sl[r["v"]:r["v"] + int(np.prod(shp))].reshape(shp).copy()
            if mm is not None:
                out[r["name"] + "_slot_m"] = mm[r["name"]]
        return out

    def optimizer_buffers(self):
        return [b for b in (self.m, self.v, self.af_slots) if b is not None]

    def view(self, buf, name):
        o = self.lay.offset[name]
        return buf[o:o + self.lay.numel(name)].view(self.lay.shape[name])

    def tview(self, name):
        o = self.lay.t_offset[name]
        r, c = self.lay.shape[name]
        return self.pbt[o:o + r * c].view(c, r)

    def load_reference_params(self, P: Dict[str, np.ndarray]):
        d, V = self.d, self.V
        with torch.no_grad():
            for name, shp in self.lay.entries:
                dst = self.view(self.p, name)
                if name.endswith("attn/qkv"):
                    base = name[:-3]
                    cat = np.concatenate([P[base + "q"], P[base + "k"], P[base + "v"]], axis=1)
                    dst.copy_(torch.from_numpy(np.ascontiguousarray(cat)))
                elif name == "to_logits/linear_out/kernel":
                    dst.zero_()
                    dst[:, :V].copy_(torch.from_numpy(np.ascontiguousarray(P[name])))
                elif name == "to_logits/linear_out/bias":
                    dst.fill_(-30000.0)
                    dst[:V].copy_(torch.from_numpy(np.ascontiguousarray(P[name])))
                else:
                    dst.copy_(torch.from_numpy(np.ascontiguousarray(P[name])).view(shp))
        self.refresh_compute_copies(cast=True)

    def export_reference(self, buf=None) -> "OrderedDict[str, np.ndarray]":
        buf = self.p if buf is None else buf
        out: "OrderedDict[str, np.ndarray]" = OrderedDict()
        d, V = self.d, self.V
        for name, shp in self.lay.entries:
            a = self.view(buf, name).detach().float().cpu().numpy()
            if name.endswith("attn/qkv"):
                base = name[:-3]
                out[base + "q"], out[base + "k"], out[base + "v"] = (np.ascontiguousarray(a[:, i * d:(i + 1) * d]) for i in range(3))
            elif name == "to_logits/linear_out/kernel":
                out[name] = np.ascontiguousarray(a[:, :V])
            elif name == "to_logits/linear_out/bias":
                out[name] = np.ascontiguousarray(a[:V])
            else:
                out[name] = a
        return out

    def init_params(self, seed=1234):
        g = torch.Generator().manual_seed(seed)
        d, L, H = self.d, self.L, self.H
        k = d // H
        P = OrderedDict()

        def nrm(shape, std):
            return (torch.randn(*shape, generator=g) * std).numpy()
        P["embedding/wte"] = nrm((self.V, d), 0.02)
        P["positional_embedding/wpe"] = nrm((self.S, d), 0.01)
        for i in range(L):
            p = f"layer_{i}/"
            P[p + "norm_1/g"], P[p + "norm_1/b"] = np.ones(d, np.float32), np.zeros(d, np.float32)
            P[p + "attn/q"] = nrm((d, d), (d * k) ** -0.5)
            P[p + "attn/k"] = nrm((d, d), d ** -0.5)
            P[p + "attn/v"] = nrm((d, d), d ** -0.5)
            P[p + "attn/o"] = nrm((d, d), (H * k) ** -0.5)
            P[p + "attn/compute_output_bias/o_b"] = np.zeros(d, np.float32)
            P[p + "norm_2/g"], P[p + "norm_2/b"] = np.ones(d, np.float32), np.zeros(d, np.float32)
            P[p + "mlp/mlp_linear_1/kernel"], P[p + "mlp/mlp_linear_1/bias"] = nrm((d, 4 * d), 0.02), np.zeros(4 * d, np.float32)
            P[p + "mlp/mlp_linear_2/kernel"], P[p + "mlp/mlp_linear_2/bias"] = nrm((4 * d, d), 0.02 / math.sqrt(L)), np.zeros(d, np.float32)
        P["to_logits/layer_norm/g"], P["to_logits/layer_norm/b"] = np.ones(d, np.float32), np.zeros(d, np.float32)
        P["to_logits/linear_out/kernel"], P["to_logits/linear_out/bias"] = nrm((d, self.V), 0.02), np.zeros(self.V, np.float32)
        self.load_reference_params(P)

    def refresh_compute_copies(self, cast=False):
        if cast:
            dh.cast_f32_bf16(self.p, self.pb, self.lay.total)
        if getattr(self, "_t_table", None) is None:
            rows, tile = [], 0
            for name in self.lay.t_offset:
                r, c = self.lay.shape[name]
                rows.append([self.lay.offset[name], self.lay.t_offset[name], r, c, tile])
                tile += ((r + 63) // 64) * ((c + 63) // 64)
            self._t_table = torch.tensor(rows, dtype=torch.int64, device=self.dev)
            self._t_tiles = tile
        dh.transpose_batch(self.pb, self.pbt, self._t_table, self._t_table.shape[0], self._t_tiles)

    def _alloc_activations(self):
        M, d, L, B, H, S, Vp = self.M, self.d, self.L, self.B, self.H, self.S, self.Vp
        b16 = dict(dtype=torch.bfloat16, device=self.dev)
        f32 = dict(dtype=torch.float32, device=self.dev)
        self.tokens = torch.zeros(B, S, dtype=torch.int32, device=self.dev)
        self.labels = torch.zeros(B, S, dtype=torch.int32, device=self.dev)
        self.X = [torch.empty(M, d, **b16) for _ in range(L + 1)]
        self.recompute = bool(self.hp.get("recompute_grad", False))
        nl = 1 if self.recompute else L

        def per_layer(make):
            bufs = [make() for _ in range(nl)]
            return [bufs[l % nl] for l in range(L)]
        self.xn1 = per_layer(lambda: torch.empty(M, d, **b16))
        self.qkv = per_layer(lambda: torch.empty(M, 3 * d, **b16))
        self.o = per_layer(lambda: torch.empty(M, d, **b16))
        self.lse = per_layer(lambda: torch.empty(B, H, S, **f32))
        self.x1 = per_layer(lambda: torch.empty(M, d, **b16))
        self.xn2 = per_layer(lambda: torch.empty(M, d, **b16))
        self.h = per_layer(lambda: torch.empty(M, 4 * d, **b16))
        gelu = self.activation == "gelu"
        self.use_relu_bits = not gelu and bool(self.hp.get("relu_bits", True)) and dh.relu_bits_auto(M, 4 * d, d)
        self.hbits = per_layer(lambda: torch.empty(dh.relu_bits_bytes(M, 4 * d), dtype=torch.uint8, device=self.dev)) if self.use_relu_bits else None
        self.hpre = per_layer(lambda: torch.empty(M, 4 * d, **b16)) if gelu else None
        self.stats = per_layer(lambda: [torch.empty(M, **f32) for _ in range(4)])
        self.xnf = torch.empty(M, d, **b16)
        self.statf = [torch.empty(M, **f32) for _ in range(2)]
        self.z = torch.empty(M, Vp, **b16)
        self.loss_rows = torch.empty(M, **f32)
        self.loss = torch.zeros(1, **f32)
        self.pos_weight = self.loss_parts = None
        if self.loss_weights is not None:
            w = position_weights(self.T, S - self.T, *self.loss_weights)
            self.pos_weight = torch.from_numpy(w.astype(np.float32)).to(self.dev)
            self.loss3 = torch.zeros(3, **f32)
            self.loss, self.loss_parts = self.loss3[0:1], self.loss3[1:3]
        self.gnorm_sq = torch.zeros(1, **f32)
        self.nparts = dh.gemm_nt_softmax_partials(Vp)
        self.zl = torch.empty(M, **f32)
        self.rowsum_part = torch.empty(self.nparts, M, **f32)
        self.rowscale = torch.empty(M, **f32)
        self.rowscale_bf = torch.empty(_round_up(M, 128) + 128, **b16)
        self.xs = torch.empty(M, d, **b16)
        self.head_flag = torch.zeros(1, dtype=torch.int32, device=self.dev)
        self.tok_sorted = torch.empty(M, dtype=torch.int32, device=self.dev)
        self.tok_perm = torch.empty(M, dtype=torch.int32, device=self.dev)
        self.sort_ws = torch.empty(dh.sort_tokens_workspace_bytes(M), dtype=torch.uint8, device=self.dev)
        self.embed_ws = torch.empty(dh.embed_bwd_workspace_bytes(B, S, d), dtype=torch.uint8, device=self.dev)
        self.sort_stream = torch.cuda.Stream(device=self.dev)
        self._sort_done = None
        self.dx = [torch.empty(M, d, **b16) for _ in range(2)]
        self.dxn = torch.empty(M, d, **b16)
        self.dh = torch.empty(M, 4 * d, **b16)
        self.dqkv = torch.empty(M, 3 * d, **b16)
        self.d_o = torch.empty(M, d, **b16)
        self.delta = torch.empty(3, B, H, S, **f32)
        wsz = max(dh.gemm_tn_workspace_bytes(M, d, Vp), dh.gemm_tn_workspace_bytes(M, 4 * d, d),
                  dh.gemm_tn_workspace_bytes(M, d, 4 * d), dh.gemm_tn_workspace_bytes(M, d, 3 * d),
                  dh.gemm_tn_workspace_bytes(M, d, d), dh.layernorm_bwd_workspace_bytes(M, d),
                  dh.sumsq_workspace_bytes(self.lay.total), dh.gemm_nt_splitk_workspace_bytes(M // 2 + 256, d, 8))
        self.ws = torch.empty(int(wsz) + 1024, dtype=torch.uint8, device=self.dev)
        self.ws_blk = [torch.empty(int(dh.gemm_tn_workspace_bytes(M, i_, j_)) + 256, dtype=torch.uint8, device=self.dev)
                       for i_, j_ in ((4 * d, d), (d, 4 * d), (d, d), (d, 3 * d))]
        self.deferred = dh.DeferredReduces()
        ln_ok = dh.gemm_nt_ln_auto(M, d, 4 * d) and self.dp_reserve_cus == 0
        self.fuse_ln = bool(self.hp.get("fuse_ln", os.environ.get("DALLE_FUSE_LN", "1") != "0")) and ln_ok
        self.fuse_ln1 = self.fuse_ln and not self.recompute
        self.hp.setdefault("dgrad_tail_split", os.environ.get("DALLE_DGRAD_TAIL", "1") != "0")
        self.hp.setdefault("defer_reduces", os.environ.get("DALLE_DEFER_REDUCES", "1") != "0")
        self.hp.setdefault("wgrad_pair", os.environ.get("DALLE_WGRAD_PAIR", "1") != "0")
        self.hp.setdefault("wgrad_group4", os.environ.get("DALLE_WGRAD_GROUP4", "1") != "0")
        self.wgrad_group4 = bool(self.hp["wgrad_group4"] and self.hp["wgrad_pair"] and self.hp["defer_reduces"]
                                 and dh.gemm_tn_group_plan([(4 * d, d), (d, 4 * d), (d, d), (d, 3 * d)], M) > 0)
        self.hp.setdefault("lnbwd_chain", os.environ.get("DALLE_LNBWD_CHAIN", "1") != "0")
        self.fuse_lnbwd = bool(self.hp.get("fuse_lnbwd", os.environ.get("DALLE_FUSE_LNBWD", "1") != "0")) and ln_ok
        if self.fuse_lnbwd:
            self.lnb_batch = bool(self.hp.get("lnbwd_batch_finish", os.environ.get("DALLE_LNBWD_BATCH", "1") != "0"))
            npart = dh.gemm_nt_lnbwd_parts(M) * 2 * d
            self.lnb_part = [torch.empty(npart, dtype=torch.float32, device=self.dev) for _ in range(2 * L if self.lnb_batch else 1)]
            self.ln_ws_final = torch.empty(int(dh.layernorm_bwd_workspace_bytes(M, d)) + 256, dtype=torch.uint8, device=self.dev)

    def _w(self, name):
        return self.view(self.pb, name)

    def forward(self, tokens: torch.Tensor, need_grad=True) -> torch.Tensor:
        M, d, L, B, H, S, Vp = self.M, self.d, self.L, self.B, self.H, self.S, self.Vp
        assert tokens.shape == (B, S) and tokens.dtype == torch.int32
        self.tokens.copy_(tokens)
        self._sort_done = None
        if need_grad:
            self._launch_sort()
        dh.shift_labels(self.tokens, self.labels, B, S, self.eos)
        dh.embed_fwd(self.tokens, self._w("embedding/wte"), self._w("positional_embedding/wpe"), self.X[0], S, d, self.V)
        for l in range(L):
            self._block_forward(l)
        if not (self.fuse_ln1 and L > 0):
            dh.layernorm_fwd(self.X[L], self._w("to_logits/layer_norm/g"), self._w("to_logits/layer_norm/b"), self.xnf,
                             self.statf[0], self.statf[1], M, d)
        Wt, bias = self.tview("to_logits/linear_out/kernel"), self._w("to_logits/linear_out/bias")
        nmb = (self.hp.get("num_microbatches", 1) or 1) if need_grad else 1
        if need_grad:
            dh.label_logit(self.xnf, d, Wt, d, bias, self.labels, self.zl, self.head_flag, M, d, self.V)
        hook = getattr(self, "event_hook", None)
        if hook is not None:
            e0 = torch.cuda.Event(enable_timing=True)
            e0.record()
        if need_grad:
            dh.gemm_nt_softmax(self.xnf, d, Wt, d, bias, None, self.z, Vp, self.rowsum_part, M, Vp, d)
        else:
            dh.gemm_nt(self.xnf, d, Wt, d, self.z, Vp, M, Vp, d, dh.GEMM_BIAS, bias=bias)
        if hook is not None:
            e1 = torch.cuda.Event(enable_timing=True)
            e1.record()
            hook().append((e0, e1))
        weighted = self.pos_weight is not None
        if need_grad and weighted:
            dh.softmax_finish_w(self.rowsum_part, self.nparts, self.zl, None, self.labels, self.xnf, d, Wt, d, bias, self.z, Vp, Vp,
                                self.loss_rows, self.rowscale, self.rowscale_bf, self.xs, self.head_flag, M, d, self.V,
                                1.0 / (self.B_global * nmb), self.pos_weight, S)
        elif need_grad:
            dh.softmax_finish(self.rowsum_part, self.nparts, self.zl, None, self.labels, self.xnf, d, Wt, d, bias, self.z, Vp, Vp,
                              self.loss_rows, self.rowscale, self.rowscale_bf, self.xs, self.head_flag, M, d, self.V,
                              1.0 / (self.B_global * S * nmb))
        else:
            dh.cross_entropy(self.z, Vp, self.labels, self.loss_rows, None, M, self.V, 0.0)
        if weighted:
            dh.loss_reduce(self.loss_rows, M, self.pos_weight, S, self.T - 1, 1.0 / (B * nmb), self.loss3)
        else:
            dh.sum_f32(self.loss_rows, M, 1.0 / (M * nmb), self.loss)
        return self.loss

    def _block_forward(self, l):
        M, d, B, H, S, L = self.M, self.d, self.B, self.H, self.S, self.L
        p = f"layer_{l}/"
        x = self.X[l]
        st = self.stats[l]
        rerun = getattr(self, "_in_backward", False)
        if not (self.fuse_ln1 and l > 0):
            dh.layernorm_fwd(x, self._w(p + "norm_1/g"), self._w(p + "norm_1/b"), self.xn1[l], st[0], st[1], M, d)
        dh.gemm_nt(self.xn1[l], d, self.tview(p + "attn/qkv"), d, self.qkv[l], 3 * d, M, 3 * d, d)
        self._attn_fwd(l, self.qkv[l], self.o[l], self.lse[l])
        if self.fuse_ln:
            dh.gemm_nt_ln(self.o[l], d, self.tview(p + "attn/o"), d, self.x1[l], d, M, d, d,
                          self._w(p + "norm_2/g"), self._w(p + "norm_2/b"), self.xn2[l], d, st[2], st[3],
                          bias=self._w(p + "attn/compute_output_bias/o_b"), residual=x)
        else:
            dh.gemm_nt(self.o[l], d, self.tview(p + "attn/o"), d, self.x1[l], d, M, d, d, dh.GEMM_BIAS | dh.GEMM_RESIDUAL,
                       bias=self._w(p + "attn/compute_output_bias/o_b"), residual=x)
            dh.layernorm_fwd(self.x1[l], self._w(p + "norm_2/g"), self._w(p + "norm_2/b"), self.xn2[l], st[2], st[3], M, d)
        if self.hpre is not None:
            dh.gemm_nt_gelu(self.xn2[l], d, self.tview(p + "mlp/mlp_linear_1/kernel"), d, self.h[l], 4 * d, M, 4 * d, d,
                            self._w(p + "mlp/mlp_linear_1/bias"), self.hpre[l], 4 * d)
        elif self.use_relu_bits:
            dh.gemm_nt_relu_bits(self.xn2[l], d, self.tview(p + "mlp/mlp_linear_1/kernel"), d, self.h[l], 4 * d, M, 4 * d, d,
                                 self._w(p + "mlp/mlp_linear_1/bias"), self.hbits[l])
        else:
            dh.gemm_nt(self.xn2[l], d, self.tview(p + "mlp/mlp_linear_1/kernel"), d, self.h[l], 4 * d, M, 4 * d, d,
                       dh.GEMM_BIAS | dh.GEMM_RELU, bias=self._w(p + "mlp/mlp_linear_1/bias"))
        if rerun:
            return
        W2, b2 = self.tview(p + "mlp/mlp_linear_2/kernel"), self._w(p + "mlp/mlp_linear_2/bias")
        if self.fuse_ln1:
            if l + 1 < L:
                q = f"layer_{l + 1}/norm_1/"
                y, mean, rstd = self.xn1[l + 1], self.stats[l + 1][0], self.stats[l + 1][1]
            else:
                q = "to_logits/layer_norm/"
                y, mean, rstd = self.xnf, self.statf[0], self.statf[1]
            dh.gemm_nt_ln(self.h[l], 4 * d, W2, 4 * d, self.X[l + 1], d, M, d, 4 * d, self._w(q + "g"), self._w(q + "b"), y, d, mean, rstd,
                          bias=b2, residual=self.x1[l])
        else:
            dh.gemm_nt(self.h[l], 4 * d, W2, 4 * d, self.X[l + 1], d, M, d, 4 * d, dh.GEMM_BIAS | dh.GEMM_RESIDUAL, bias=b2, residual=self.x1[l])

    def logits(self) -> torch.Tensor:
        return self.z.view(self.B, self.S, self.Vp)[:, :, :self.V].float()

    def sample_image_tokens(self, text: torch.Tensor, temperature: float = 1.0, top_k: int = 0, seed: int = 0,
                            top_p: float = 1.0, image_prefix: Optional[torch.Tensor] = None, return_logprobs: bool = False,
                            kv_cache: bool = True, decode_graph: bool = True, fused_sampling: bool = True,
                            guidance_scale: float = 1.0, uncond_text: Optional[torch.Tensor] = None):
        B, T, S, P = self.B, self.T, self.S, self.S - self.T
        gs = float(guidance_scale)
        if not (gs >= 0.0 and math.isfinite(gs)):
            raise ValueError(f"sample_image_tokens: guidance_scale must be finite and >= 0 (got {guidance_scale})")
        guided = gs != 1.0 or uncond_text is not None
        R = B
        if guided:
            if B % 2:
                raise ValueError(f"sample_image_tokens: guidance pairs the engine's rows, so its batch must be even (B = {B})")
            R = B // 2
            if tuple(text.shape) != (R, T):
                raise ValueError(f"sample_image_tokens: with guidance text must be [B / 2 = {R}, T = {T}] (got {tuple(text.shape)})")
            if uncond_text is None:
                pad = self.hp.get("padding_id")
                uncond_text = torch.full((T,), self.text_vocab_size - 1 if pad is None else int(pad), dtype=torch.int32)
            uncond_text = torch.as_tensor(uncond_text)
            if uncond_text.dtype.is_floating_point or uncond_text.dtype == torch.bool:
                raise ValueError("sample_image_tokens: uncond_text must hold integer token ids")
            if tuple(uncond_text.shape) not in ((T,), (R, T)):
                raise ValueError(f"sample_image_tokens: uncond_text must be [T = {T}] or [B / 2 = {R}, T = {T}] "
                                 f"(got {tuple(uncond_text.shape)})")
            if int(uncond_text.min()) < 0 or int(uncond_text.max()) >= self.text_vocab_size:
                raise ValueError(f"sample_image_tokens: uncond_text ids must lie in [0, {self.text_vocab_size})")
        assert text.shape == (R, T)
        top_p = float(top_p)
        if not (0.0 < top_p <= 1.0):
            raise ValueError(f"sample_image_tokens: top_p must lie in (0, 1] (got {top_p})")
        lo, hi = self.text_vocab_size, self.text_vocab_size + self.image_vocab_size
        nv = hi - lo
        k = 0
        if image_prefix is not None:
            image_prefix = torch.as_tensor(image_prefix)
            if image_prefix.dim() != 2 or image_prefix.shape[0] != R or not (0 <= image_prefix.shape[1] < P):
                raise ValueError(f"sample_image_tokens: image_prefix must be [B={R}, k] with 0 <= k < {P} (got {tuple(image_prefix.shape)})")
            if image_prefix.dtype.is_floating_point or image_prefix.dtype == torch.bool:
                raise ValueError("sample_image_tokens: image_prefix must hold integer token ids")
            k = int(image_prefix.shape[1])
            if k and (int(image_prefix.min()) < 0 or int(image_prefix.max()) >= nv):
                raise ValueError(f"sample_image_tokens: image_prefix ids must lie in [0, {nv})")
        nucleus = top_p < 1.0 or return_logprobs
        toks = torch.full((B, S), lo, dtype=torch.int32, device=self.dev)
# ... 116 lines not shown
        D["pos_i"][0:1].fill_(pos)
        self._run_decode(sample=False, graph=graph)
        return D["logits"]

    def _run_decode(self, sample, graph: bool):
        D = self._dec
        if not graph:
            self._decode_body(sample)
        elif sample not in D["graphs"] and sample not in D["warm"]:
            self._decode_body(sample)
            D["warm"].add(sample)
        else:
            if sample not in D["graphs"]:
                torch.cuda.synchronize()
                g = torch.cuda.CUDAGraph()
                with _no_gc_in_capture(), torch.cuda.graph(g, capture_error_mode="thread_local"):
                    self._decode_body(sample)
                D["graphs"][sample] = g
            D["graphs"][sample].replay()

    def _decode_body(self, sample=False):
        B, d, L, H, S = self.B, self.d, self.L, self.H, self.S
        D = self._dec
        x, x1, xn, o, h, st, z, fresh = D["x"][0], D["x"][1], D["xn"], D["o"], D["h"], D["st"], D["z"], D["fresh"]
        fuse_ln = B <= 32 and d <= 2048 and self.image_vocab_size % 16 == 0 and self.hp.get("decode_fuse_ln", True)

        def ln_dense(inp, ln, W, out, N, flags=0, bias=None):
            g, b = self._w(ln + "/g"), self._w(ln + "/b")
            if fuse_ln:
                dh.ln_gemm_nt(inp, d, g, b, W, d, out, N, B, N, d, flags, bias=bias)
            else:
                dh.layernorm_fwd(inp, g, b, xn, st[0], st[1], B, d)
                dh.gemm_nt(xn, d, W, d, out, N, B, N, d, flags, bias=bias)

        act = dh.GEMM_GELU if self.activation == "gelu" else dh.GEMM_RELU
        caches = self._kv_caches()
        dh.embed_fwd(D["tok"], self._w("embedding/wte"), self._w("positional_embedding/wpe"), x, S, d, self.V,
                     pos_dev=D["pos_i"])
        for l in range(L):
            p = f"layer_{l}/"
            cache = caches[l]
            ln_dense(x, p + "norm_1", self.tview(p + "attn/qkv"), fresh, 3 * d)
            if self.attn_plan[l] is None:
                dh.attention_decode(cache, o, B, H, S, 0, fresh=fresh, pos_dev=D["pos_i"], head_dim=self.hd)
            else:
                dh.attention_decode_masked(cache, o, self.attn_plan[l], B, H, S, 0, fresh=fresh, pos_dev=D["pos_i"], head_dim=self.hd)
            dh.gemm_nt(o, d, self.tview(p + "attn/o"), d, x1, d, B, d, d, dh.GEMM_BIAS | dh.GEMM_RESIDUAL,
                       bias=self._w(p + "attn/compute_output_bias/o_b"), residual=x)
            ln_dense(x1, p + "norm_2", self.tview(p + "mlp/mlp_linear_1/kernel"), h, 4 * d, dh.GEMM_BIAS | act,
                     bias=self._w(p + "mlp/mlp_linear_1/bias"))
            dh.gemm_nt(h, 4 * d, self.tview(p + "mlp/mlp_linear_2/kernel"), 4 * d, x, d, B, d, 4 * d,
                       dh.GEMM_BIAS | dh.GEMM_RESIDUAL, bias=self._w(p + "mlp/mlp_linear_2/bias"), residual=x1)
        lo, nv = self.text_vocab_size, self.image_vocab_size
        Wt = self.tview("to_logits/linear_out/kernel")
        ln_dense(x, "to_logits/layer_norm", Wt[lo:lo + nv], z, nv)
        bias = self._w("to_logits/linear_out/bias")[lo:lo + nv]
        if sample in ("g", "g+logp"):
            dh.sample_tokens_guided(z, nv, bias, B // 2, nv, params_dev=D["params"], pos_dev=D["pos_i"], advance=True, token_offset=lo,
                                    next_tok=D["tok"], out=D["out"], out_col0=self.T - 1, logp=D["logp"] if sample == "g+logp" else None)
        elif sample in ("p", "p+logp"):
            dh.sample_tokens_p(z, nv, bias, B, nv, params_dev=D["params"], pos_dev=D["pos_i"], advance=True, token_offset=lo,
                               next_tok=D["tok"], out=D["out"], out_col0=self.T - 1, logp=D["logp"] if sample == "p+logp" else None)
        elif sample:
            dh.sample_tokens(z, nv, bias, B, nv, params_dev=D["params"], pos_dev=D["pos_i"], advance=True, token_offset=lo,
                             next_tok=D["tok"], out=D["out"], out_col0=self.T - 1)
        else:
            dh.logits_f32(z, nv, bias, D["logits"], B, nv)

    def _gv(self, name):
        return self.view(self.g, name)

    def _wgrad(self, X, ldx, dY, ldy, dW, M, I, J, dbias=None, bias_weights=None, slot=None):
        if slot is None or not self.hp["defer_reduces"]:
            dh.gemm_tn(X, ldx, dY, ldy, dW, M, I, J, self.ws, dbias=dbias, bias_weights=bias_weights)
        else:
            dh.gemm_tn(X, ldx, dY, ldy, dW, M, I, J, self.ws_blk[slot], dbias=dbias, bias_weights=bias_weights,
                       deferred=self.deferred)

    def _launch_sort(self):
        main = torch.cuda.current_stream()
        self.sort_stream.wait_stream(main)
        with torch.cuda.stream(self.sort_stream):
            dh.sort_tokens(self.tokens, self.tok_sorted, self.tok_perm, self.M, self.V, self.sort_ws)
            self._sort_done = torch.cuda.Event()
            self._sort_done.record(self.sort_stream)

    def backward(self, allreduce=True):
        reserve = self.dp_reserve_cus if allreduce else 0
        if not reserve:
            return self._backward(allreduce)
        dh.set_option("reserve_cus", reserve)
        try:
            return self._backward(allreduce)
        finally:
            dh.set_option("reserve_cus", 0)

    def _backward(self, allreduce):
        M, d, L, B, H, S, Vp = self.M, self.d, self.L, self.B, self.H, self.S, self.Vp
        ws = self.ws
        E = self.z
        rp = self.lay.ready_points
        done = [0]

        def ready(upto):
            if allreduce:
                self.reducer.ready(done[0], upto)
            done[0] = upto

        if self._sort_done is None:
            self._launch_sort()
        self._wgrad(self.xs, d, E, Vp, self._gv("to_logits/linear_out/kernel"), M, d, Vp,
                    dbias=self._gv("to_logits/linear_out/bias"), bias_weights=self.rowscale_bf)
        ready(rp[0])
        Wk = self._w("to_logits/linear_out/kernel")
        tn8 = (d + 255) // 256
        whole_rows = min(M, (((M + 255) // 256) * tn8 // 256) * 256 // tn8 * 256) if self.hp["dgrad_tail_split"] else M
        if whole_rows in (0, M) or Vp < 8192:
            dh.gemm_nt(E, Vp, Wk, Vp, self.dxn, d, M, d, Vp, dh.GEMM_ROWSCALE, rowscale=self.rowscale)
        else:
            tail_rows = M - whole_rows
            tail_tiles = ((tail_rows + 255) // 256) * tn8
            ns = next((k for k in (2, 4, 8) if (tail_tiles * k) % 256 == 0 and Vp // k >= 4096), 2)
            dh.gemm_nt(E, Vp, Wk, Vp, self.dxn, d, whole_rows, d, Vp, dh.GEMM_ROWSCALE, rowscale=self.rowscale)
            dh.gemm_nt_splitk(E[whole_rows:], Vp, Wk, Vp, self.dxn[whole_rows:], tail_rows, d, Vp, ns, self.ws,
                              rowscale=self.rowscale[whole_rows:])
        dxa, dxb = self.dx
        pend = []

        def ln_bwd(idx, dy, x, g, mean, rstd, dres, dx, dg, db):
            if self.fuse_lnbwd and self.lnb_batch and idx == 2 * L:
                dh.layernorm_bwd(dy, x, g, mean, rstd, dres, dx, None, None, self.ln_ws_final, M, d)
                pend.append((self.ln_ws_final, dg, db, M))
            else:
                dh.layernorm_bwd(dy, x, g, mean, rstd, dres, dx, dg, db, ws, M, d)

        def flush_ln():
            while pend:
                dh.layernorm_bwd_finish_batch(pend[:16], d)
                del pend[:16]

        def lnbwd(idx, A, K, Wn, x, g, mean, rstd, dres, dx, dg, db, B2=None, C2=None):
            kw = dict(B2=B2, ldb2=d, C2=C2) if B2 is not None else {}
            if self.lnb_batch:
                part = self.lnb_part[idx]
                dh.gemm_nt_lnbwd(A, K, Wn, K, M, d, K, x, g, mean, rstd, dres, dx, part, **kw)
                pend.append((part, dg, db, 32 * dh.gemm_nt_lnbwd_parts(M)))
            else:
                dh.gemm_nt_lnbwd(A, K, Wn, K, M, d, K, x, g, mean, rstd, dres, dx, self.lnb_part[0], dg=dg, db=db, **kw)

        ln_bwd(2 * L, self.dxn, self.X[L], self._w("to_logits/layer_norm/g"), self.statf[0], self.statf[1], None, dxa,
               self._gv("to_logits/layer_norm/g"), self._gv("to_logits/layer_norm/b"))
        for bi, l in enumerate(reversed(range(L))):
            p = f"layer_{l}/"
            st = self.stats[l]
            if self.recompute:
                self._in_backward = True
                self._block_forward(l)
                self._in_backward = False
            pair = self.hp["wgrad_pair"] and self.hp["defer_reduces"]
            group4 = pair and self.wgrad_group4
            if not group4:
                self._wgrad(self.h[l], 4 * d, dxa, d, self._gv(p + "mlp/mlp_linear_2/kernel"), M, 4 * d, d,
                            dbias=self._gv(p + "mlp/mlp_linear_2/bias"), slot=0)
            if self.hpre is not None:
                dh.gemm_nt_gelu_grad(dxa, d, self._w(p + "mlp/mlp_linear_2/kernel"), d, self.dh, 4 * d, M, 4 * d, d, self.hpre[l], 4 * d)
            elif self.use_relu_bits:
                dh.gemm_nt_mask_bits(dxa, d, self._w(p + "mlp/mlp_linear_2/kernel"), d, self.dh, 4 * d, M, 4 * d, d, self.hbits[l])
            else:
                dh.gemm_nt(dxa, d, self._w(p + "mlp/mlp_linear_2/kernel"), d, self.dh, 4 * d, M, 4 * d, d, dh.GEMM_RELU_MASK,
                           relu_src=self.h[l])
            if not group4:
                self._wgrad(self.xn2[l], d, self.dh, 4 * d, self._gv(p + "mlp/mlp_linear_1/kernel"), M, d, 4 * d,
                            dbias=self._gv(p + "mlp/mlp_linear_1/bias"), slot=1)
            chain = self.fuse_lnbwd and self.hp["lnbwd_chain"]
            if self.fuse_lnbwd:
                lnbwd(2 * l + 1, self.dh, 4 * d, self._w(p + "mlp/mlp_linear_1/kernel"), self.x1[l], self._w(p + "norm_2/g"), st[2], st[3],
                      dxa, dxb, self._gv(p + "norm_2/g"), self._gv(p + "norm_2/b"),
                      B2=self._w(p + "attn/o") if chain else None, C2=self.d_o if chain else None)
            else:
                dh.gemm_nt(self.dh, 4 * d, self._w(p + "mlp/mlp_linear_1/kernel"), 4 * d, self.dxn, d, M, d, 4 * d)
                ln_bwd(2 * l + 1, self.dxn, self.x1[l], self._w(p + "norm_2/g"), st[2], st[3], dxa, dxb,
                       self._gv(p + "norm_2/g"), self._gv(p + "norm_2/b"))
            if not pair:
                self._wgrad(self.o[l], d, dxb, d, self._gv(p + "attn/o"), M, d, d,
                            dbias=self._gv(p + "attn/compute_output_bias/o_b"), slot=2)
            if not chain:
                dh.gemm_nt(dxb, d, self._w(p + "attn/o"), d, self.d_o, d, M, d, d)
            if self.attn_plan[l] is None:
                dh.attention_bwd(self.qkv[l], self.o[l], self.d_o, self.lse[l], self.delta, self.dqkv, B, H, S, head_dim=self.hd)
            else:
                dh.attention_bwd_masked(self.qkv[l], self.o[l], self.d_o, self.lse[l], self.delta, self.dqkv, self.attn_plan[l],
                                        B, H, S, head_dim=self.hd)
            if pair:
                probs = [dict(X=self.o[l], ldx=d, dY=dxb, ldy=d, dW=self._gv(p + "attn/o"), I=d, J=d, ws=self.ws_blk[2],
                              dbias=self._gv(p + "attn/compute_output_bias/o_b")),
                         dict(X=self.xn1[l], ldx=d, dY=self.dqkv, ldy=3 * d, dW=self._gv(p + "attn/qkv"), I=d, J=3 * d, ws=self.ws_blk[3])]
                if group4:
                    probs = [dict(X=self.h[l], ldx=4 * d, dY=dxa, ldy=d, dW=self._gv(p + "mlp/mlp_linear_2/kernel"), I=4 * d, J=d,
                                  ws=self.ws_blk[0], dbias=self._gv(p + "mlp/mlp_linear_2/bias")),
                             dict(X=self.xn2[l], ldx=d, dY=self.dh, ldy=4 * d, dW=self._gv(p + "mlp/mlp_linear_1/kernel"), I=d, J=4 * d,
                                  ws=self.ws_blk[1], dbias=self._gv(p + "mlp/mlp_linear_1/bias"))] + probs
                dh.gemm_tn_group(probs, M, deferred=self.deferred)
            else:
                self._wgrad(self.xn1[l], d, self.dqkv, 3 * d, self._gv(p + "attn/qkv"), M, d, 3 * d, slot=3)
            if self.fuse_lnbwd:
                lnbwd(2 * l, self.dqkv, 3 * d, self._w(p + "attn/qkv"), self.X[l], self._w(p + "norm_1/g"), st[0], st[1],
                      dxb, dxa, self._gv(p + "norm_1/g"), self._gv(p + "norm_1/b"))
            else:
                dh.gemm_nt(self.dqkv, 3 * d, self._w(p + "attn/qkv"), 3 * d, self.dxn, d, M, d, 3 * d)
                ln_bwd(2 * l, self.dxn, self.X[l], self._w(p + "norm_1/g"), st[0], st[1], dxb, dxa,
                       self._gv(p + "norm_1/g"), self._gv(p + "norm_1/b"))
            self.deferred.run()
            if allreduce and self.world > 1:
                flush_ln()
            ready(rp[1 + bi])
        if self._sort_done is not None:
            torch.cuda.current_stream().wait_event(self._sort_done)
        dh.embed_bwd(self.tok_sorted, self.tok_perm, dxa, self._gv("embedding/wte"), self._gv("positional_embedding/wpe"),
                     B, S, d, self.V, self.embed_ws)
        flush_ln()
        ready(rp[L + 1])

    def wait_grads(self):
        self.reducer.finish()

    def learning_rate(self, step=None) -> float:
        hp = self.hp
        step = self.global_step if step is None else step
        lr0 = hp["lr"]
        end = hp.get("lr_decay_end") or hp["train_steps"]
        decay = hp.get("lr_decay", "cosine") or "cosine"
        warm = hp.get("warmup_steps", 3000)
        warm = 3000 if warm is None else warm
        f32 = np.float32
        s = min(step, end)
        if decay == "linear":
            v = f32((lr0 - lr0 * 0.1) * (1.0 - s / end) + lr0 * 0.1)
        elif decay == "cosine":
            v = f32(lr0 * ((1.0 - 0.1) * 0.5 * (1.0 + math.cos(math.pi * s / end)) + 0.1))
        else:
            v = f32(lr0)
        if warm > 0 and step < warm:
            v = f32(v * f32(f32(step) / f32(warm)))
        return float(v)

    def optimizer_step(self):
        self.wait_grads()
        if self.optimizer == "adafactor":
            return self._adafactor_step()
        return self._adam_step()

    def _adafactor_step(self):
        hp = self.hp
        clip = hp.get("gradient_clipping", 1.0)
        lr = self.learning_rate()
        get = lambda k, dflt: dflt if hp.get(k) is None else float(hp[k])
        if self._af_beta1() != 0.0 and self.m is None:
            self.m = torch.zeros(self.lay.total, dtype=torch.float32, device=self.dev)
        dh.adafactor_step(self.af_table, len(self.af_vars), self.af_totals, self.p, self.g, self.m, self.af_slots, self.pb,
                          self.gnorm_sq, 0.0 if clip is None else float(clip), lr, get("weight_decay", 0.0), self._af_beta1(),
                          get("epsilon_1", 1e-30), get("epsilon_2", 1e-3), self.af_ws)
        self.refresh_compute_copies(cast=False)
        self.global_step += 1
        return lr

    def _adam_step(self):
        hp = self.hp
        n = self.lay.total
        clip = hp.get("gradient_clipping", 1.0)
        lr = self.learning_rate()
        b1 = hp.get("beta_1") or 0.9
        b2 = hp.get("beta_2") or 0.999
        eps = hp.get("epsilon") or 1e-6
        wd = hp.get("weight_decay") or 0.0
        gn = None
        cl = 0.0
        if clip is not None:
            dh.sumsq(self.g, n, self.gnorm_sq, self.ws)
            gn, cl = self.gnorm_sq, float(clip)
        if not wd:
            dh.adam_step(self.p, self.g, self.m, self.v, self.pb, n, gn, cl, lr, b1, b2, eps, 0.0)
        else:
            for name, _ in self.lay.entries:
                o, k = self.lay.offset[name], _round_up(self.lay.numel(name), ALIGN)
                use = ("norm" not in name) and ("bias" not in name) and not name.endswith("o_b")
                dh.adam_step(self.p[o:o + k], self.g[o:o + k], self.m[o:o + k], self.v[o:o + k], self.pb[o:o + k], k, gn, cl,
                             lr, b1, b2, eps, wd if use else 0.0)
        self.refresh_compute_copies(cast=False)
        self.global_step += 1
        return lr

    def train_step(self, tokens: torch.Tensor) -> torch.Tensor:
        nmb = self.hp.get("num_microbatches", 1) or 1
        if nmb == 1:
            loss = self.forward(tokens, need_grad=True)
            self.backward()
            self.optimizer_step()
            return loss
        assert tokens.shape == (nmb * self.B, self.S), f"expected {nmb} micro-batches of {self.B} rows"
        if getattr(self, "gacc", None) is None:
            self.gacc = torch.empty_like(self.g)
        if getattr(self, "loss_acc", None) is None:
            self.loss_acc = torch.zeros_like(self.loss)
        self.loss_acc.zero_()
        if self.loss_parts is not None:
            if getattr(self, "loss_parts_acc", None) is None:
                self.loss_parts_acc = torch.zeros_like(self.loss_parts)
            self.loss_parts_acc.zero_()
        for i in range(nmb):
            loss = self.forward(tokens[i * self.B:(i + 1) * self.B], need_grad=True)
            self.loss_acc += loss
            if self.loss_parts is not None:
                self.loss_parts_acc.add_(self.loss_parts, alpha=1.0 / nmb)
            self.backward(allreduce=False)
            if i == 0:
                self.gacc.copy_(self.g)
            else:
                dh.add_f32(self.gacc, self.g, self.lay.total)
        self.g.copy_(self.gacc)
        self.reducer.ready(0, self.lay.total)
        self.optimizer_step()
        return self.loss_acc

    def grad_norm(self) -> float:
        return float(torch.sqrt(self.gnorm_sq).item())

    def state_dict(self):
        sd = {"p": self.p.detach().cpu(), "global_step": self.global_step, "optimizer": self.optimizer, "activation_fn": self.activation}
        for k in ("m", "v", "af_slots"):
            if getattr(self, k) is not None:
                sd[k] = getattr(self, k).detach().cpu()
        return sd

    def load_state_dict(self, sd):
        written = sd.get("optimizer", "adam")
        if written != self.optimizer:
            raise ValueError(f"checkpoint was written by the {written} optimizer; this run uses {self.optimizer}: "
                             "the optimizer state of one cannot continue the other")
        act = sd.get("activation_fn", "relu")
        if act != self.activation:
            raise ValueError(f"checkpoint was written by a {act} model; this run uses activation_fn {self.activation!r}: "
                             "the weights of one do not compute the other")
        self.p.copy_(sd["p"])
        for k in ("m", "v", "af_slots"):
            if getattr(self, k) is not None:
                if k not in sd:
                    raise ValueError(f"checkpoint has no {k!r} state for {self.optimizer} (beta_1 differs from the run's?)")
                getattr(self, k).copy_(sd[k])
        self.global_step = int(sd["global_step"])
        self.refresh_compute_copies(cast=True)
```

### include/dalle_hip.h

```cpp
#ifndef DALLE_HIP_H
#define DALLE_HIP_H
#include <stddef.h>
#include <stdint.h>
#ifdef __cplusplus
extern "C" {
#endif

typedef enum {
  DMI_OK = 0,
  DMI_ERR_INVALID = -1,
  DMI_ERR_LAUNCH = -2,
  DMI_ERR_UNSUPPORTED = -3
} dmi_status;

const char* dmi_last_error_string(void);
int dmi_version(void);
int dmi_get_option(const char* name);
int dmi_set_option(const char* name, int value);
int dmi_set_debug_buffer(void* device_buffer);

int dmi_embed_fwd(const int32_t* tokens, const uint16_t* wte, const uint16_t* wpe, uint16_t* x,
                  int64_t rows , int S, int d, int vocab, const int* pos_dev, void* stream);
int64_t dmi_sort_tokens_workspace_bytes(int64_t n);
int dmi_sort_tokens(const int32_t* tokens, int32_t* sorted_tokens, int32_t* perm, int64_t n, int vocab,
                    void* workspace, void* stream);
int64_t dmi_embed_bwd_workspace_bytes(int B, int S, int d);
int dmi_embed_bwd(const int32_t* sorted_tokens, const int32_t* perm, const uint16_t* dx, float* dwte,
                  float* dwpe, int B, int S, int d, int vocab, void* workspace, void* stream);

int dmi_layernorm_fwd(const uint16_t* x, const uint16_t* g, const uint16_t* b, uint16_t* y,
                      float* mean, float* rstd, int64_t rows, int d, float eps, void* stream);
int64_t dmi_layernorm_bwd_workspace_bytes(int64_t rows, int d);
int dmi_layernorm_bwd(const uint16_t* dy, const uint16_t* x, const uint16_t* g, const float* mean,
                      const float* rstd, const uint16_t* dres, uint16_t* dx, float* dg, float* db,
                      void* workspace, int64_t rows, int d, void* stream);
int dmi_layernorm_bwd_finish_batch(const void* const* workspaces, float* const* dgs, float* const* dbs, const int64_t* rows,
                                   int n, int d, void* stream);

#define DMI_GEMM_BIAS 1
#define DMI_GEMM_RELU 2
#define DMI_GEMM_RESIDUAL 4
#define DMI_GEMM_RELU_MASK 8
#define DMI_GEMM_OUT_F32 16
#define DMI_GEMM_ROWSCALE 32
#define DMI_GEMM_GELU 512
int dmi_gemm_nt(const uint16_t* A, int lda, const uint16_t* Bt, int ldb, void* C, int ldc,
                int M, int N, int K, int flags, const uint16_t* bias, const uint16_t* residual,
                const uint16_t* relu_src, const float* rowscale, void* stream);
int dmi_ln_gemm_nt(const uint16_t* X, int ldx, const uint16_t* gamma, const uint16_t* beta, float eps, const uint16_t* Bt, int ldb,
                   uint16_t* C, int ldc, int M, int N, int K, int flags, const uint16_t* bias, void* stream);
int64_t dmi_gemm_nt_splitk_workspace_bytes(int M, int N, int nsplit);
int dmi_gemm_nt_splitk(const uint16_t* A, int lda, const uint16_t* Bt, int ldb, uint16_t* C, int M, int N, int K,
                       int nsplit, const float* rowscale, void* workspace, void* stream);
int64_t dmi_gemm_tn_workspace_bytes(int M, int I, int J);
typedef struct dmi_reduce_item { const float* slabs; float* out; int nsplit; int64_t n4; } dmi_reduce_item;
int dmi_gemm_tn(const uint16_t* X, int ldx, const uint16_t* dY, int ldy, float* dW, float* dbias,
                const uint16_t* bias_weights, int M, int I, int J, void* workspace, dmi_reduce_item* deferred,
                int* n_deferred, void* stream);
int dmi_reduce_slabs_batch(const dmi_reduce_item* items, int n, void* stream);
typedef struct dmi_tn_problem { const uint16_t* X; int ldx; const uint16_t* dY; int ldy; float* dW; float* dbias;
                                const uint16_t* bias_weights; int I; int J; void* workspace; } dmi_tn_problem;
int dmi_gemm_tn_group(const dmi_tn_problem* probs, int n, int M, dmi_reduce_item* deferred, int* n_deferred, void* stream);
int dmi_gemm_tn_group_plan(const int* I, const int* J, int n, int M);

int64_t dmi_colsum_workspace_bytes(int64_t M, int N);
int dmi_colsum(const uint16_t* Y, int ldy, float* out, int64_t M, int N, void* workspace, void* stream);
int dmi_transpose_bf16(const uint16_t* in, uint16_t* out, int batch, int R, int C, void* stream);

int dmi_attention_fwd(const uint16_t* qkv, uint16_t* o, float* lse, int B, int H, int S, void* stream);
int dmi_attention_bwd(const uint16_t* qkv, const uint16_t* o, const uint16_t* d_o, const float* lse, float* scratch,
                      uint16_t* dqkv, int B, int H, int S, void* stream);

int dmi_attention_decode(uint16_t* qkv, const uint16_t* fresh, uint16_t* o, int B, int H, int S, int pos, const int* pos_dev,
                         void* stream);
int dmi_attention_fwd_hd(const uint16_t* qkv, uint16_t* o, float* lse, int B, int H, int S, int head_dim, void* stream);
int dmi_attention_bwd_hd(const uint16_t* qkv, const uint16_t* o, const uint16_t* d_o, const float* lse, float* scratch,
                         uint16_t* dqkv, int B, int H, int S, int head_dim, void* stream);
int dmi_attention_decode_hd(uint16_t* qkv, const uint16_t* fresh, uint16_t* o, int B, int H, int S, int pos, const int* pos_dev,
                            int head_dim, void* stream);

int64_t dmi_attn_mask_plan(const uint8_t* mask, int S, int32_t* plan, int64_t plan_bytes);
int dmi_attention_fwd_masked(const uint16_t* qkv, uint16_t* o, float* lse, const int32_t* plan, const int32_t* plan_host, int B, int H,
                             int S, int head_dim, void* stream);
int dmi_attention_bwd_masked(const uint16_t* qkv, const uint16_t* o, const uint16_t* d_o, const float* lse, float* scratch,
                             uint16_t* dqkv, const int32_t* plan, const int32_t* plan_host, int B, int H, int S, int head_dim,
                             void* stream);
int dmi_attention_decode_masked(uint16_t* qkv, const uint16_t* fresh, uint16_t* o, const int32_t* plan, const int32_t* plan_host,
                                int B, int H, int S, int pos, const int* pos_dev, int head_dim, void* stream);

int dmi_shift_labels(const int32_t* tokens, int32_t* labels, int B, int S, int eos, void* stream);
int dmi_cross_entropy(uint16_t* z, int ldz, const int32_t* labels, float* loss_rows, float* lse,
                      int64_t M, int V, float dz_scale, void* stream);
int dmi_label_logit(const uint16_t* X, int ldx, const uint16_t* Wt, int ldw, const uint16_t* bias,
                    const int32_t* labels, float* zl, int32_t* flag, int64_t M, int K, int V, void* stream);
int64_t dmi_gemm_nt_softmax_partials(int N);
int dmi_gemm_nt_ln(const uint16_t* A, int lda, const uint16_t* Bt, int ldb, uint16_t* C, int ldc, int M, int N, int K,
                   const uint16_t* bias, const uint16_t* residual, const uint16_t* gamma, const uint16_t* beta, float eps,
                   uint16_t* Y, int ldy, float* mean, float* rstd, void* stream);
int64_t dmi_relu_bits_bytes(int M, int N);
int dmi_relu_bits_auto(int M, int N, int K);
int dmi_gemm_nt_relu_bits(const uint16_t* A, int lda, const uint16_t* Bt, int ldb, uint16_t* C, int ldc, int M, int N, int K,
                          const uint16_t* bias, void* bits, void* stream);
int dmi_gemm_nt_mask_bits(const uint16_t* A, int lda, const uint16_t* Bt, int ldb, uint16_t* C, int ldc, int M, int N, int K,
                          const void* bits, void* stream);
int dmi_gemm_nt_gelu(const uint16_t* A, int lda, const uint16_t* Bt, int ldb, uint16_t* C, int ldc, int M, int N, int K,
                     const uint16_t* bias, uint16_t* pre, int ldpre, void* stream);
int dmi_gemm_nt_gelu_grad(const uint16_t* A, int lda, const uint16_t* Bt, int ldb, uint16_t* C, int ldc, int M, int N, int K,
                          const uint16_t* pre, int ldpre, void* stream);
int dmi_gemm_nt_lnbwd_parts(int M);
int dmi_gemm_nt_ln_auto(int M, int N, int K);
int dmi_gemm_nt_lnbwd(const uint16_t* A, int lda, const uint16_t* Bt, int ldb, int M, int N, int K, const uint16_t* x,
                      const uint16_t* gamma, const float* mean, const float* rstd, const uint16_t* dres, uint16_t* dx,
                      float* part, const uint16_t* B2, int ldb2, uint16_t* C2, void* stream);
int dmi_layernorm_bwd_finish_parts(const float* part, int P, float* dg, float* db, int d, void* stream);
int dmi_gemm_nt_softmax(const uint16_t* X, int ldx, const uint16_t* Wt, int ldw, const uint16_t* bias,
                        const float* rowshift, uint16_t* E, int lde, float* rowsum_part, int M, int N, int K, void* stream);
int dmi_softmax_finish(const float* rowsum_part, int nparts, const float* label_logit, const float* rowshift,
                       const int32_t* labels, const uint16_t* X, int ldx,
                       const uint16_t* Wt, int ldw, const uint16_t* bias, uint16_t* E, int lde, int N,
                       float* loss_rows, float* rowscale, uint16_t* rowscale_bf16, uint16_t* Xs, int32_t* flag,
                       int64_t M, int K, int V, float dz_scale, void* stream);
int dmi_sum_f32(const float* x, int64_t n, float scale, float* out, void* stream);
int dmi_softmax_finish_w(const float* rowsum_part, int nparts, const float* label_logit, const float* rowshift,
                         const int32_t* labels, const uint16_t* X, int ldx,
                         const uint16_t* Wt, int ldw, const uint16_t* bias, uint16_t* E, int lde, int N,
                         float* loss_rows, float* rowscale, uint16_t* rowscale_bf16, uint16_t* Xs, int32_t* flag,
                         int64_t M, int K, int V, float dz_scale, const float* pos_weight, int period, void* stream);
int dmi_loss_reduce(const float* loss_rows, int64_t M, const float* pos_weight, int period, int split, float scale,
                    float* out3, void* stream);

int dmi_assemble_tokens(const int32_t* text, const float* vae_logits, int32_t* tokens_out,
                        int B, int T, int P, int C, int text_vocab, void* stream);

int dmi_sample_tokens(const uint16_t* z, int ldz, const uint16_t* bias, int B, int nv, float temperature, int top_k,
                      uint64_t seed, const uint32_t* params_dev, int pos, int32_t* pos_dev, int advance, int token_offset,
                      int32_t* next_tok, int32_t* out, int out_ld, int out_col0, void* stream);

int dmi_sample_tokens_p(const uint16_t* z, int ldz, const uint16_t* bias, int B, int nv, float temperature, int top_k,
                        uint64_t seed, float top_p, const uint32_t* params_dev, int pos, int32_t* pos_dev, int advance,
                        int token_offset, int32_t* next_tok, int32_t* out, int out_ld, int out_col0, float* logp, void* stream);

int dmi_sample_tokens_guided(const uint16_t* z, int ldz, const uint16_t* bias, int Bc, int nv, float temperature, int top_k,
                             uint64_t seed, float top_p, float scale, const uint32_t* params_dev, int pos, int32_t* pos_dev,
                             int advance, int token_offset, int32_t* next_tok, int32_t* out, int out_ld, int out_col0, float* logp,
                             void* stream);

int dmi_logits_f32(const uint16_t* z, int ldz, const uint16_t* bias, float* out, int B, int nv, void* stream);

int64_t dmi_sumsq_workspace_bytes(int64_t n);
int dmi_sumsq(const float* g, int64_t n, float* out, void* workspace, void* stream);
int dmi_adam_step(float* p, const float* g, float* m, float* v, uint16_t* p_bf16, int64_t n,
                  const float* gnorm_sq, float clip, float lr, float beta1, float beta2, float eps,
                  float weight_decay, float grad_scale, const float* lr_dev, void* stream);

#define DMI_AF_FIELDS 17
int dmi_adafactor_plan(int64_t* table, int nvars, int64_t* totals);
int dmi_adafactor_step(const int64_t* table_dev, int nvars, const int64_t* totals, float* p, const float* g, float* m,
                       float* slots, uint16_t* p_bf16, float* gnorm_sq, float clip, float lr, const float* lr_dev,
                       float decay, float beta1, float eps1, float eps2, void* workspace, int64_t workspace_bytes, void* stream);

int dmi_comm_load(const char* librccl_path);
int dmi_comm_unique_id_bytes(void);
int dmi_comm_unique_id(void* id_out);
int dmi_comm_init(void** comm_out, int nranks, int rank, const void* unique_id);
int dmi_comm_destroy(void* comm);
int dmi_allreduce_bucket(void* comm, float* g, int64_t n, void* stream);
int dmi_comm_broadcast_f32(void* comm, float* buf, int64_t n, int root, void* stream);

int dmi_cast_f32_bf16(const float* in, uint16_t* out, int64_t n, void* stream);

int dmi_transpose_bf16_batch(const uint16_t* in_base, uint16_t* out_base, const int64_t* table, int n,
                             int64_t total_tiles, void* stream);

int dmi_transpose_bf16_padded(const uint16_t* in, uint16_t* out, int R_valid, int R_pitch, int C, void* stream);

int dmi_conv_gemm_nt(const uint16_t* x, int B, int H, int W, int C, int Ho, int Wo, int stride, int ntaps,
                     const int* dy, const int* dx, const uint16_t* Wt, int ldw, uint16_t* out, int ldc, int N,
                     int flags, const uint16_t* bias, const uint16_t* residual, const uint16_t* relu_src, void* stream);

int64_t dmi_conv_wgrad_tn_workspace_bytes(int M, int K, int N);
int dmi_conv_wgrad_tn(const uint16_t* x, int B, int H, int W, int C, int Ho, int Wo, int stride, int ntaps,
                      const int* dy, const int* dx, const uint16_t* dY, int ldy, int N, float* dW, float* dbias,
                      void* workspace, dmi_reduce_item* deferred, int* n_deferred, void* stream);

int dmi_im2col(const uint16_t* x, uint16_t* out, int B, int H, int W, int C, int Ho, int Wo, int stride,
               int ntaps, const int* dy, const int* dx, int ldo, void* stream);
int dmi_weight_gather(const uint16_t* in, uint16_t* out, int A, int Bn, int nsel, const int* idx, int ldo, void* stream);
int dmi_weight_gather_batch(const uint16_t* in_base, uint16_t* out_base, const int64_t* table, int n, int64_t total_blocks,
                            void* stream);
int dmi_pixel_interleave(const uint16_t* in4, uint16_t* out, int B, int Ht, int Wt, int C, void* stream);
int dmi_pad_channels(const float* in, uint16_t* out, int64_t N, int Cin, int Cp, void* stream);
int dmi_unpad_channels(const uint16_t* in, float* out, int64_t N, int Cin, int Cp, void* stream);
int dmi_conv2d_f32(const float* x, int B, int H, int W, int C, int Ho, int Wo, int stride, int ntaps, const int* dy,
                   const int* dx, const float* Wk, const float* bias, const float* residual, float* out, int N, int relu,
                   void* stream);
int dmi_space_to_depth_f32(const float* img, float* stacked, int B, int Hs, int Ws, int C, int s, int Cp, void* stream);
int dmi_depth_to_space_f32(const float* stacked, float* img, int B, int Hs, int Ws, int C, int s, int Cp, void* stream);
int dmi_gumbel_softmax_fwd(const float* logits, const float* u, uint16_t* y, uint16_t* y_soft, int32_t* index,
                           int64_t M, int T, float temperature, int hard, const float* temperature_dev, void* stream);
int dmi_gumbel_softmax_bwd(const uint16_t* dy, const uint16_t* y_soft, uint16_t* dlogits, int64_t M, int T,
                           float temperature, const float* temperature_dev, void* stream);
int64_t dmi_mse_workspace_bytes(void);
int dmi_mse_loss(const float* img, const uint16_t* outp, uint16_t* dout, float* loss, int64_t N, int Cin, int Cp,
                 float grad_scale, void* workspace, void* stream);
int dmi_add_f32(float* dst, const float* src, int64_t n, void* stream);


uint32_t dmi_crc32c(const void* data, size_t n);

#ifdef __cplusplus
}
#endif
#endif
```

Baseline: 2.824 million.

## Fuse embed+LN, fold label logit into softmax finish, early wte zero, transposed Adam

Adds a fused kernel that computes the embedding sum, shift labels, resets the flag, and applies the first layer's LayerNorm in a single pass. It also folds the label-logit dot product into the softmax-finish kernel, which removes a separate launch. The wte gradient memset moves onto the sort side stream so it overlaps other work. Adam gains a variant that writes transposed bf16 weights directly, avoiding a separate transpose pass. These are several independent launch-count and memory-traffic reductions behind env-controlled flags that default to on. The cost is more code paths and extra per-block work inside softmax_finish.

```diff
diff --git a/dalle-mtf_amd/csrc/elementwise.hip b/dalle-mtf_amd/csrc/elementwise.hip
--- a/dalle-mtf_amd/csrc/elementwise.hip
+++ b/dalle-mtf_amd/csrc/elementwise.hip
@@ -251,14 +251,14 @@
 extern "C" int64_t dmi_embed_bwd_workspace_bytes(int B, int S, int d) {
   return (((int64_t)B * S + EB_CH - 1) / EB_CH) * 2 * d * 4 + 256;
 }
-extern "C" int dmi_embed_bwd(const int32_t* sorted_tokens, const int32_t* perm, const uint16_t* dx, float* dwte,
-                             float* dwpe, int B, int S, int d, int vocab, void* workspace, void* stream) {
+static int embed_bwd_launch(const int32_t* sorted_tokens, const int32_t* perm, const uint16_t* dx, float* dwte,
+                            float* dwpe, int B, int S, int d, int vocab, void* workspace, bool fill, void* stream) {
   DMI_REQUIRE(sorted_tokens && perm && dx && dwte && dwpe && workspace, "embed_bwd: null pointer");
   DMI_REQUIRE(d % 8 == 0 && B > 0 && S > 0 && vocab > 0, "embed_bwd: bad sizes");
   hipStream_t st = (hipStream_t)stream;
   embed_bwd_wpe_kernel<<<dim3((S + 3) / 4), dim3(256), 0, st>>>(dx, dwpe, B, S, d);
   DMI_CHECK_LAUNCH("embed_bwd_wpe");
-  DMI_REQUIRE(hipMemsetAsync(dwte, 0, (size_t)vocab * d * 4, st) == hipSuccess, "embed_bwd: memset failed");
+  if (fill) DMI_REQUIRE(hipMemsetAsync(dwte, 0, (size_t)vocab * d * 4, st) == hipSuccess, "embed_bwd: memset failed");
   const int64_t n = (int64_t)B * S;
   const int64_t chunks = cdiv64(n, EB_CH);
   embed_bwd_wte_sorted_kernel<<<dim3((unsigned)cdiv64(chunks, 4)), dim3(256), 0, st>>>(sorted_tokens, perm, dx, dwte, (float*)workspace, n, d, vocab);
@@ -266,6 +266,55 @@
   embed_bwd_wte_combine_kernel<<<dim3((unsigned)cdiv64(chunks, 4)), dim3(256), 0, st>>>(sorted_tokens, dwte, (const float*)workspace, n, d, vocab);
   DMI_CHECK_LAUNCH("embed_bwd_wte_combine");
   return DMI_OK;
+}
+extern "C" int dmi_embed_bwd(const int32_t* sorted_tokens, const int32_t* perm, const uint16_t* dx, float* dwte,
+                             float* dwpe, int B, int S, int d, int vocab, void* workspace, void* stream) {
+  return embed_bwd_launch(sorted_tokens, perm, dx, dwte, dwpe, B, S, d, vocab, workspace, true, stream);
+}
+extern "C" int dmi_embed_bwd_zero(float* dwte, int d, int vocab, void* stream) {
+  DMI_REQUIRE(dwte && d > 0 && vocab > 0, "embed_bwd_zero: bad args");
+  DMI_REQUIRE(hipMemsetAsync(dwte, 0, (size_t)vocab * d * 4, (hipStream_t)stream) == hipSuccess, "embed_bwd_zero: memset failed");
+  return DMI_OK;
+}
+extern "C" int dmi_embed_bwd_zeroed(const int32_t* sorted_tokens, const int32_t* perm, const uint16_t* dx, float* dwte,
+                                    float* dwpe, int B, int S, int d, int vocab, void* workspace, void* stream) {
+  return embed_bwd_launch(sorted_tokens, perm, dx, dwte, dwpe, B, S, d, vocab, workspace, false, stream);
+}
+
+template <int NC>
+__device__ __forceinline__ void ln_row_finish(float (&v)[NC][8], float sum, int lane, int nch, int d, float eps,
+                                              const bf16_t* __restrict__ g, const bf16_t* __restrict__ b, bf16_t* __restrict__ yrow,
+                                              float* __restrict__ mean_row, float* __restrict__ rstd_row) {
+  const float mu = wave_sum(sum) / (float)d;
+  float sq = 0.f;
+#pragma unroll
+  for (int i = 0; i < NC; ++i) {
+    const int c = lane + 64 * i;
+    if (c < nch) {
+#pragma unroll
+      for (int j = 0; j < 8; ++j) {
+        v[i][j] -= mu;
+        sq += v[i][j] * v[i][j];
+      }
+    }
+  }
+  const float rs = rsqrtf(wave_sum(sq) / (float)d + eps);
+#pragma unroll
+  for (int i = 0; i < NC; ++i) {
+    const int c = lane + 64 * i;
+    if (c < nch) {
+      float fg[8], fb[8], o[8];
+      unpack8(*(const u32x4*)(g + c * 8), fg);
+      unpack8(*(const u32x4*)(b + c * 8), fb);
+#pragma unroll
+      for (int j = 0; j < 8; ++j) o[j] = v[i][j] * rs * fg[j] + fb[j];
+      *(u32x4*)(yrow + c * 8) = pack8(o);
+    }
+  }
+  if (lane == 0) {
+    *mean_row = mu;
+    *rstd_row = rs;
+  }
 }
 
 template <int NC>
@@ -288,36 +337,46 @@
       for (int j = 0; j < 8; ++j) sum += v[i][j];
     }
   }
-  const float mu = wave_sum(sum) / (float)d;
-  float sq = 0.f;
+  ln_row_finish<NC>(v, sum, lane, nch, d, eps, g, b, y + row * d, mean + row, rstd + row);
+}
+
+template <int NC>
+__global__ __launch_bounds__(256) void embed_fwd_ln_kernel(const int* __restrict__ tokens, const bf16_t* __restrict__ wte,
+                                                           const bf16_t* __restrict__ wpe, bf16_t* __restrict__ x,
+                                                           int64_t rows, int S, int d, int vocab,
+                                                           const bf16_t* __restrict__ g, const bf16_t* __restrict__ b,
+                                                           bf16_t* __restrict__ y, float* __restrict__ mean, float* __restrict__ rstd,
+                                                           float eps, int* __restrict__ labels, int eos, int* __restrict__ flag) {
+  const int lane = threadIdx.x & 63, wid = threadIdx.x >> 6;
+  if (flag && blockIdx.x == 0 && threadIdx.x == 0) flag[0] = 0;
+  const int64_t row = (int64_t)blockIdx.x * 4 + wid;
+  if (row >= rows) return;
+  int tok = tokens[row];
+  tok = tok < 0 ? 0 : (tok >= vocab ? vocab - 1 : tok);
+  const int s = (int)(row % S);
+  if (labels && lane == 0) labels[row] = (s == S - 1) ? eos : tokens[row + 1];
+  const bf16_t* a = wte + (int64_t)tok * d;
+  const bf16_t* p = wpe + (int64_t)s * d;
+  const int nch = d / 8;
+  float v[NC][8];
+  float sum = 0.f;
 #pragma unroll
   for (int i = 0; i < NC; ++i) {
     const int c = lane + 64 * i;
     if (c < nch) {
-#pragma unroll
-      for (int j = 0; j < 8; ++j) {
-        v[i][j] -= mu;
-        sq += v[i][j] * v[i][j];
-      }
-    }
-  }
-  const float rs = rsqrtf(wave_sum(sq) / (float)d + eps);
-#pragma unroll
-  for (int i = 0; i < NC; ++i) {
-    const int c = lane + 64 * i;
-    if (c < nch) {
-      float fg[8], fb[8], o[8];
-      unpack8(*(const u32x4*)(g + c * 8), fg);
-      unpack8(*(const u32x4*)(b + c * 8), fb);
-#pragma unroll
-      for (int j = 0; j < 8; ++j) o[j] = v[i][j] * rs * fg[j] + fb[j];
-      *(u32x4*)(y + row * d + c * 8) = pack8(o);
-    }
-  }
-  if (lane == 0) {
-    mean[row] = mu;
-    rstd[row] = rs;
-  }
+      float fa[8], fp[8];
+      unpack8(*(const u32x4*)(a + c * 8), fa);
+      unpack8(*(const u32x4*)(p + c * 8), fp);
+#pragma unroll
+      for (int j = 0; j < 8; ++j) fa[j] += fp[j];
+      const u32x4 o = pack8(fa);
+      *(u32x4*)(x + row * d + c * 8) = o;
+      unpack8(o, v[i]);
+#pragma unroll
+      for (int j = 0; j < 8; ++j) sum += v[i][j];
+    }
+  }
+  ln_row_finish<NC>(v, sum, lane, nch, d, eps, g, b, y + row * d, mean + row, rstd + row);
 }
 
 extern "C" int dmi_layernorm_fwd(const uint16_t* x, const uint16_t* g, const uint16_t* b, uint16_t* y, float* mean,
@@ -331,6 +390,25 @@
   else if (d <= 2048) ln_fwd_kernel<4><<<grid, blk, 0, st>>>(x, g, b, y, mean, rstd, rows, d, eps);
   else ln_fwd_kernel<8><<<grid, blk, 0, st>>>(x, g, b, y, mean, rstd, rows, d, eps);
   DMI_CHECK_LAUNCH("layernorm_fwd");
+  return DMI_OK;
+}
+
+extern "C" int dmi_embed_fwd_ln(const int32_t* tokens, const uint16_t* wte, const uint16_t* wpe, uint16_t* x, int64_t rows, int S,
+                                int d, int vocab, const uint16_t* g, const uint16_t* b, uint16_t* y, float* mean, float* rstd,
+                                float eps, int32_t* labels, int eos, int32_t* flag, void* stream) {
+  DMI_REQUIRE(tokens && wte && wpe && x && g && b && y && mean && rstd, "embed_fwd_ln: null pointer");
+  DMI_REQUIRE(d % 8 == 0 && d <= 4096 && rows > 0 && S > 0 && vocab > 0, "embed_fwd_ln: unsupported sizes (d=%d: need d%%8==0, d<=4096; rows=%lld)",
+              d, (long long)rows);
+  DMI_REQUIRE(!labels || rows % S == 0, "embed_fwd_ln: labels need whole sequences (rows %% S == 0)");
+  hipStream_t st = (hipStream_t)stream;
+  dim3 grid((unsigned)cdiv64(rows, 4)), blk(256);
+#define EFL_ARGS tokens, wte, wpe, x, rows, S, d, vocab, g, b, y, mean, rstd, eps, labels, eos, flag
+  if (d <= 512) embed_fwd_ln_kernel<1><<<grid, blk, 0, st>>>(EFL_ARGS);
+  else if (d <= 1024) embed_fwd_ln_kernel<2><<<grid, blk, 0, st>>>(EFL_ARGS);
+  else if (d <= 2048) embed_fwd_ln_kernel<4><<<grid, blk, 0, st>>>(EFL_ARGS);
+  else embed_fwd_ln_kernel<8><<<grid, blk, 0, st>>>(EFL_ARGS);
+#undef EFL_ARGS
+  DMI_CHECK_LAUNCH("embed_fwd_ln");
   return DMI_OK;
 }
 
@@ -620,6 +698,23 @@
   return DMI_OK;
 }
 
+__device__ __forceinline__ void transpose_tile_store(bf16_t* __restrict__ dst, int R, int C, int r0, int c0, unsigned (*t)[33]) {
+  const int tid = threadIdx.x;
+  const int orow = tid >> 2, seg = tid & 3;
+  const int c = c0 + orow, r = r0 + 16 * seg;
+  if (c < C) {
+#pragma unroll
+    for (int q = 0; q < 2; ++q) {
+      const int rr = r + 8 * q;
+      if (rr < R) {
+        u32x4 v;
+#pragma unroll
+        for (int i = 0; i < 4; ++i) v[i] = t[orow][8 * seg + 4 * q + i];
+        *(u32x4*)(dst + (int64_t)c * R + rr) = v;
+      }
+    }
+  }
+}
 __device__ __forceinline__ void transpose_tile(const bf16_t* __restrict__ src, bf16_t* __restrict__ dst, int Rv, int R,
                                                int C, int64_t sr, int r0, int c0, unsigned (*t)[33]) {
   const int tid = threadIdx.x;
@@ -639,22 +734,7 @@
     }
   }
   __syncthreads();
-  {
-    const int orow = tid >> 2, seg = tid & 3;
-    const int c = c0 + orow, r = r0 + 16 * seg;
-    if (c < C) {
-#pragma unroll
-      for (int q = 0; q < 2; ++q) {
-        const int rr = r + 8 * q;
-        if (rr < R) {
-          u32x4 v;
-#pragma unroll
-          for (int i = 0; i < 4; ++i) v[i] = t[orow][8 * seg + 4 * q + i];
-          *(u32x4*)(dst + (int64_t)c * R + rr) = v;
-        }
-      }
-    }
-  }
+  transpose_tile_store(dst, R, C, r0, c0, t);
 }
 
 __global__ __launch_bounds__(256) void transpose_kernel(const bf16_t* __restrict__ in, bf16_t* __restrict__ out,
@@ -964,12 +1044,53 @@
 #define SF_PARTS 16
 struct NoWeight { static constexpr bool on = false; };
 struct PosWeight { static constexpr bool on = true; const float* w; int period; };
-template <class PW>
-__global__ __launch_bounds__(256) void softmax_finish_kernel(SoftmaxFinishArgs a, PW pw) {
+struct NoLabelLogit { static constexpr bool on = false; };
+struct LabelLogit { static constexpr bool on = true; const bf16_t* Wt; int ldw; const bf16_t* bias; float* zl; };
+template <class PW, class ZL>
+__global__ __launch_bounds__(256) void softmax_finish_kernel(SoftmaxFinishArgs a, PW pw, ZL zq) {
   __shared__ float sm[SF_PARTS][SF_ROWS];
   __shared__ float sc[SF_ROWS];
   const int tid = threadIdx.x, r4 = tid & 15, q = tid >> 4;
   const int64_t m0 = (int64_t)blockIdx.x * SF_ROWS, m = m0 + 4 * r4;
+  __shared__ float szl[ZL::on ? SF_ROWS : 1];
+  if constexpr (ZL::on) {
+    const int lane = tid & 63, wid = tid >> 6;
+    for (int r0 = 16 * wid; r0 < 16 * wid + 16 && m0 + r0 < a.M; r0 += 4) {
+      int64_t mr[4];
+      int lab[4];
+      float acc[4] = {0.f, 0.f, 0.f, 0.f};
+#pragma unroll
+      for (int u = 0; u < 4; ++u) {
+        mr[u] = m0 + r0 + u < a.M ? m0 + r0 + u : a.M - 1;
+        const int l = a.labels[mr[u]];
+        lab[u] = l < 0 ? 0 : (l >= a.V ? a.V - 1 : l);
+      }
+      for (int c = lane; c < a.K / 8; c += 64) {
+        u32x4 xa[4], wb[4];
+#pragma unroll
+        for (int u = 0; u < 4; ++u) {
+          xa[u] = *(const u32x4*)(a.X + mr[u] * a.ldx + c * 8);
+          wb[u] = *(const u32x4*)(zq.Wt + (int64_t)lab[u] * zq.ldw + c * 8);
+        }
+#pragma unroll
+        for (int u = 0; u < 4; ++u) {
+          float fa[8], fb[8];
+          unpack8(xa[u], fa);
+          unpack8(wb[u], fb);
+#pragma unroll
+          for (int j = 0; j < 8; ++j) acc[u] = __builtin_fmaf(fa[j], fb[j], acc[u]);
+        }
+      }
+#pragma unroll
+      for (int u = 0; u < 4; ++u) {
+        const float z = wave_sum(acc[u]) + bf2f(zq.bias[lab[u]]);
+        if (lane == 0 && m0 + r0 + u < a.M) {
+          szl[r0 + u] = z;
+          zq.zl[m0 + r0 + u] = z;
+        }
+      }
+    }
+  }
   f32x4 s = {0.f, 0.f, 0.f, 0.f};
   if (m + 3 < a.M && (a.M & 3) == 0) {
     for (int p = q; p < a.nparts; p += SF_PARTS) {
@@ -994,7 +1115,9 @@
       for (int k = 0; k < SF_PARTS; ++k) S += sm[k][r];
       const bool bad = !(S > 1.0e-18f && S < 1.0e18f);
       if (bad) a.flag[0] = 1;
-      a.loss_rows[mr] = bad ? INFINITY : __logf(S) + (a.rowshift ? a.rowshift[mr] : 0.f) - a.zl[mr];
+      float zl;
+      if constexpr (ZL::on) zl = szl[r]; else zl = a.zl[mr];
+      a.loss_rows[mr] = bad ? INFINITY : __logf(S) + (a.rowshift ? a.rowshift[mr] : 0.f) - zl;
       float dz = a.dz_scale;
       if constexpr (PW::on) dz *= pw.w[(int)(((int64_t)(m0 % pw.period) + r) % pw.period)];
       scale = bad ? 0.f : dz / S;
@@ -1092,11 +1215,12 @@
       }
   }
 }
-static int softmax_finish_launch(const float* rowsum_part, int nparts, const float* label_logit, const float* rowshift,
+static int softmax_finish_launch(const float* rowsum_part, int nparts, const float* label_logit_in, const float* rowshift,
                                  const int32_t* labels, const uint16_t* X, int ldx,
                                  const uint16_t* Wt, int ldw, const uint16_t* bias, uint16_t* E, int lde, int N,
                                  float* loss_rows, float* rowscale, uint16_t* rowscale_bf16, uint16_t* Xs, int32_t* flag,
-                                 int64_t M, int K, int V, float dz_scale, const float* pos_weight, int period, void* stream) {
+                                 int64_t M, int K, int V, float dz_scale, const float* pos_weight, int period, float* zl_out, void* stream) {
+  const float* label_logit = label_logit_in ? label_logit_in : zl_out;
   DMI_REQUIRE(rowsum_part && label_logit && labels && X && Wt && bias && E && loss_rows && flag, "softmax_finish: null pointer");
   DMI_REQUIRE(dz_scale == 0.f || (rowscale && rowscale_bf16 && Xs), "softmax_finish: gradient outputs missing");
   DMI_REQUIRE(M > 0 && K % 8 == 0 && K <= FIX_MAXK && ldx % 8 == 0 && ldw % 8 == 0 && nparts > 0 && V > 0 && V <= N && N <= lde,
@@ -1107,8 +1231,12 @@
   a.M = M; a.K = K; a.V = V; a.dz_scale = dz_scale;
   hipStream_t st = (hipStream_t)stream;
   const PosWeight pw{pos_weight, period};
-  if (pos_weight) softmax_finish_kernel<<<dim3((unsigned)cdiv64(M, SF_ROWS)), dim3(256), 0, st>>>(a, pw);
-  else softmax_finish_kernel<<<dim3((unsigned)cdiv64(M, SF_ROWS)), dim3(256), 0, st>>>(a, NoWeight{});
+  const dim3 grid((unsigned)cdiv64(M, SF_ROWS)), blk(256);
+  const LabelLogit zq{Wt, ldw, bias, zl_out};
+  if (zl_out && pos_weight) softmax_finish_kernel<<<grid, blk, 0, st>>>(a, pw, zq);
+  else if (zl_out) softmax_finish_kernel<<<grid, blk, 0, st>>>(a, NoWeight{}, zq);
+  else if (pos_weight) softmax_finish_kernel<<<grid, blk, 0, st>>>(a, pw, NoLabelLogit{});
+  else softmax_finish_kernel<<<grid, blk, 0, st>>>(a, NoWeight{}, NoLabelLogit{});
   DMI_CHECK_LAUNCH("softmax_finish");
   if (pos_weight) softmax_fixup_kernel<<<dim3(256), dim3(256), 0, st>>>(a, Wt, ldw, bias, N, pw);
   else softmax_fixup_kernel<<<dim3(256), dim3(256), 0, st>>>(a, Wt, ldw, bias, N, NoWeight{});
@@ -1121,7 +1249,7 @@
                                   float* loss_rows, float* rowscale, uint16_t* rowscale_bf16, uint16_t* Xs, int32_t* flag,
                                   int64_t M, int K, int V, float dz_scale, void* stream) {
   return softmax_finish_launch(rowsum_part, nparts, label_logit, rowshift, labels, X, ldx, Wt, ldw, bias, E, lde, N, loss_rows, rowscale,
-                               rowscale_bf16, Xs, flag, M, K, V, dz_scale, nullptr, 0, stream);
+                               rowscale_bf16, Xs, flag, M, K, V, dz_scale, nullptr, 0, nullptr, stream);
 }
 extern "C" int dmi_softmax_finish_w(const float* rowsum_part, int nparts, const float* label_logit, const float* rowshift,
                                     const int32_t* labels, const uint16_t* X, int ldx,
@@ -1131,7 +1259,17 @@
   DMI_REQUIRE(pos_weight, "softmax_finish_w: null pos_weight");
   DMI_REQUIRE(period > 0, "softmax_finish_w: period must be > 0");
   return softmax_finish_launch(rowsum_part, nparts, label_logit, rowshift, labels, X, ldx, Wt, ldw, bias, E, lde, N, loss_rows, rowscale,
-                               rowscale_bf16, Xs, flag, M, K, V, dz_scale, pos_weight, period, stream);
+                               rowscale_bf16, Xs, flag, M, K, V, dz_scale, pos_weight, period, nullptr, stream);
+}
+extern "C" int dmi_softmax_finish_zl(const float* rowsum_part, int nparts, float* label_logit, const int32_t* labels,
+                                     const uint16_t* X, int ldx, const uint16_t* Wt, int ldw, const uint16_t* bias, uint16_t* E,
+                                     int lde, int N, float* loss_rows, float* rowscale, uint16_t* rowscale_bf16, uint16_t* Xs,
+                                     int32_t* flag, int64_t M, int K, int V, float dz_scale, const float* pos_weight, int period,
+                                     void* stream) {
+  DMI_REQUIRE(label_logit, "softmax_finish_zl: null label_logit");
+  DMI_REQUIRE(!pos_weight || period > 0, "softmax_finish_zl: period must be > 0");
+  return softmax_finish_launch(rowsum_part, nparts, nullptr, nullptr, labels, X, ldx, Wt, ldw, bias, E, lde, N, loss_rows, rowscale,
+                               rowscale_bf16, Xs, flag, M, K, V, dz_scale, pos_weight, period, label_logit, stream);
 }
 
 __device__ __forceinline__ float block_sum_256(float x, float* sm) {
@@ -1249,6 +1387,33 @@
   return DMI_OK;
 }
 
+__device__ __forceinline__ u32x2 adam_update4(float* __restrict__ p, const float* __restrict__ g, float* __restrict__ m,
+                                              float* __restrict__ v, int64_t i, float mult, float lr, float b1, float b2, float eps,
+                                              float wd) {
+  f32x4 pv = ((f32x4*)p)[i], gv = ((const f32x4*)g)[i], mv = ((f32x4*)m)[i], vv = ((f32x4*)v)[i];
+#pragma unroll
+  for (int j = 0; j < 4; ++j) {
+    const float gg = gv[j] * mult;
+    mv[j] = b1 * mv[j] + (1.f - b1) * gg;
+    vv[j] = b2 * vv[j] + (1.f - b2) * gg * gg;
+    float upd = mv[j] / (sqrtf(vv[j]) + eps);
+    upd += wd * pv[j];
+    pv[j] -= lr * upd;
+  }
+  ((f32x4*)p)[i] = pv;
+  ((f32x4*)m)[i] = mv;
+  ((f32x4*)v)[i] = vv;
+  return u32x2{pack2bf(pv[0], pv[1]), pack2bf(pv[2], pv[3])};
+}
+__device__ __forceinline__ float adam_mult(const float* __restrict__ gnorm_sq, float clip, float gscale) {
+  float mult = gscale;
+  if (gnorm_sq != nullptr && clip > 0.f) {
+    const float gn = sqrtf(gnorm_sq[0]) * gscale;
+    mult = gscale * (clip / fmaxf(gn, clip));
+  }
+  return mult;
+}
+
 __global__ __launch_bounds__(256) void adam_kernel(float* __restrict__ p, const float* __restrict__ g,
                                                    float* __restrict__ m, float* __restrict__ v,
                                                    bf16_t* __restrict__ pb, int64_t n,
@@ -1256,27 +1421,11 @@
                                                    float b2, float eps, float wd, float gscale,
                                                    const float* __restrict__ lr_dev) {
   if (lr_dev) lr = lr_dev[0];
-  float mult = gscale;
-  if (gnorm_sq != nullptr && clip > 0.f) {
-    const float gn = sqrtf(gnorm_sq[0]) * gscale;
-    mult = gscale * (clip / fmaxf(gn, clip));
-  }
+  const float mult = adam_mult(gnorm_sq, clip, gscale);
   const int64_t n4 = n / 4;
   for (int64_t i = (int64_t)blockIdx.x * 256 + threadIdx.x; i < n4; i += (int64_t)gridDim.x * 256) {
-    f32x4 pv = ((f32x4*)p)[i], gv = ((const f32x4*)g)[i], mv = ((f32x4*)m)[i], vv = ((f32x4*)v)[i];
-#pragma unroll
-    for (int j = 0; j < 4; ++j) {
-      const float gg = gv[j] * mult;
-      mv[j] = b1 * mv[j] + (1.f - b1) * gg;
-      vv[j] = b2 * vv[j] + (1.f - b2) * gg * gg;
-      float upd = mv[j] / (sqrtf(vv[j]) + eps);
-      upd += wd * pv[j];
-      pv[j] -= lr * upd;
-    }
-    ((f32x4*)p)[i] = pv;
-    ((f32x4*)m)[i] = mv;
-    ((f32x4*)v)[i] = vv;
-    if (pb) *(u32x2*)(pb + i * 4) = u32x2{pack2bf(pv[0], pv[1]), pack2bf(pv[2], pv[3])};
+    const u32x2 r = adam_update4(p, g, m, v, i, mult, lr, b1, b2, eps, wd);
+    if (pb) *(u32x2*)(pb + i * 4) = r;
   }
   if (blockIdx.x == 0 && threadIdx.x < (n & 3)) {
     const int64_t i = n4 * 4 + threadIdx.x;
@@ -1301,6 +1450,97 @@
   if (blocks > 4096) blocks = 4096;
   adam_kernel<<<dim3((unsigned)blocks), dim3(256), 0, (hipStream_t)stream>>>(p, g, m, v, p_bf16, n, gnorm_sq, clip, lr, beta1, beta2, eps, weight_decay, grad_scale, lr_dev);
   DMI_CHECK_LAUNCH("adam_step");
+  return DMI_OK;
+}
+
+#define ADAMT_CHUNK 4096
+__global__ __launch_bounds__(256) void adam_kernel_t(float* __restrict__ p, const float* __restrict__ g, float* __restrict__ m,
+                                                     float* __restrict__ v, bf16_t* __restrict__ pb, bf16_t* __restrict__ pbt,
+                                                     int64_t n, const int64_t* __restrict__ table, int ntab, int64_t total_tiles,
+                                                     const float* __restrict__ gnorm_sq, float clip, float lr, float b1, float b2,
+                                                     float eps, float wd, float gscale, const float* __restrict__ lr_dev) {
+  __shared__ unsigned t[64][33];
+  if (lr_dev) lr = lr_dev[0];
+  const float mult = adam_mult(gnorm_sq, clip, gscale);
+  const int tid = threadIdx.x;
+  if ((int64_t)blockIdx.x < total_tiles) {
+    const int64_t tile = blockIdx.x;
+    int i = 0;
+    while (i + 1 < ntab && table[(i + 1) * 5 + 4] <= tile) ++i;
+    const int64_t in_off = table[i * 5], out_off = table[i * 5 + 1];
+    const int R = (int)table[i * 5 + 2], C = (int)table[i * 5 + 3];
+    const int local = (int)(tile - table[i * 5 + 4]);
+    const int tc = (C + 63) / 64;
+    const int r0 = (local / tc) * 64, c0 = (local % tc) * 64;
+    const int chunk = tid & 7, rp = tid >> 3;
+    const int ra = r0 + 2 * rp, c = c0 + 8 * chunk;
+    u32x4 va = {0, 0, 0, 0}, vb = {0, 0, 0, 0};
+    if (c < C) {
+#pragma unroll
+      for (int h = 0; h < 2; ++h) {
+        if (ra + h < R) {
+          const int64_t e = in_off + (int64_t)(ra + h) * C + c;
+          const u32x2 lo = adam_update4(p, g, m, v, e / 4, mult, lr, b1, b2, eps, wd);
+          const u32x2 hi = adam_update4(p, g, m, v, e / 4 + 1, mult, lr, b1, b2, eps, wd);
+          const u32x4 w = {lo[0], lo[1], hi[0], hi[1]};
+          *(u32x4*)(pb + e) = w;
+          if (h == 0) va = w; else vb = w;
+        }
+      }
+    }
+#pragma unroll
+    for (int j = 0; j < 8; ++j) {
+      const unsigned lo = (va[j >> 1] >> ((j & 1) * 16)) & 0xffffu;
+      const unsigned hi = (vb[j >> 1] >> ((j & 1) * 16)) & 0xffffu;
+      t[8 * chunk + j][rp] = lo | (hi << 16);
+    }
+    __syncthreads();
+    transpose_tile_store(pbt + out_off, R, C, r0, c0, t);
+    return;
+  }
+  const int64_t lo = ((int64_t)blockIdx.x - total_tiles) * ADAMT_CHUNK;
+  const int64_t hi = lo + ADAMT_CHUNK < n ? lo + ADAMT_CHUNK : n;
+  int i0 = 0;
+  while (i0 < ntab && table[i0 * 5] + table[i0 * 5 + 2] * table[i0 * 5 + 3] <= lo) ++i0;
+  if (i0 < ntab && table[i0 * 5] <= lo && table[i0 * 5] + table[i0 * 5 + 2] * table[i0 * 5 + 3] >= hi) return;
+  const int64_t n4 = n / 4;
+#pragma unroll
+  for (int k = 0; k < ADAMT_CHUNK / 1024; ++k) {
+    const int64_t i = lo / 4 + k * 256 + tid;
+    if (i >= n4 || i * 4 >= hi) continue;
+    bool inside = false;
+    for (int q = i0; q < ntab && table[q * 5] < hi; ++q)
+      inside = inside || (i * 4 >= table[q * 5] && i * 4 < table[q * 5] + table[q * 5 + 2] * table[q * 5 + 3]);
+    if (inside) continue;
+    const u32x2 r = adam_update4(p, g, m, v, i, mult, lr, b1, b2, eps, wd);
+    *(u32x2*)(pb + i * 4) = r;
+  }
+  if (hi == n && tid < (n & 3)) {
+    const int64_t e = n4 * 4 + tid;
+    const float gg = g[e] * mult;
+    const float mm = b1 * m[e] + (1.f - b1) * gg;
+    const float vv = b2 * v[e] + (1.f - b2) * gg * gg;
+    float pp = p[e];
+    pp -= lr * (mm / (sqrtf(vv) + eps) + wd * pp);
+    p[e] = pp;
+    m[e] = mm;
+    v[e] = vv;
+    pb[e] = f2bf(pp);
+  }
+}
+extern "C" int dmi_adam_step_t(float* p, const float* g, float* m, float* v, uint16_t* p_bf16, uint16_t* pt_bf16, int64_t n,
+                               const int64_t* table, int ntab, int64_t total_tiles, const float* gnorm_sq, float clip, float lr,
+                               float beta1, float beta2, float eps, float weight_decay, float grad_scale, const float* lr_dev,
+                               void* stream) {
+  DMI_REQUIRE(p && g && m && v && p_bf16 && pt_bf16 && table && n > 0 && ntab > 0 && total_tiles > 0, "adam_step_t: bad args");
+  DMI_REQUIRE((((uintptr_t)p | (uintptr_t)g | (uintptr_t)m | (uintptr_t)v | (uintptr_t)p_bf16 | (uintptr_t)pt_bf16) & 15) == 0,
+              "adam_step_t: buffers must be 16-byte aligned");
+  const int64_t blocks = total_tiles + cdiv64(n, ADAMT_CHUNK);
+  DMI_REQUIRE(blocks < 0x7fffffff, "adam_step_t: too many blocks");
+  adam_kernel_t<<<dim3((unsigned)blocks), dim3(256), 0, (hipStream_t)stream>>>(p, g, m, v, p_bf16, pt_bf16, n, table, ntab, total_tiles,
+                                                                               gnorm_sq, clip, lr, beta1, beta2, eps, weight_decay,
+                                                                               grad_scale, lr_dev);
+  DMI_CHECK_LAUNCH("adam_step_t");
   return DMI_OK;
 }
 
diff --git a/dalle-mtf_amd/dalle_hip/__init__.py b/dalle-mtf_amd/dalle_hip/__init__.py
--- a/dalle-mtf_amd/dalle_hip/__init__.py
+++ b/dalle-mtf_amd/dalle_hip/__init__.py
@@ -58,6 +58,9 @@
         "dmi_sort_tokens": (I, [P, P, P, L64, I, P, P]),
         "dmi_embed_bwd_workspace_bytes": (L64, [I, I, I]),
         "dmi_embed_bwd": (I, [P, P, P, P, P, I, I, I, I, P, P]),
+        "dmi_embed_bwd_zero": (I, [P, I, I, P]),
+        "dmi_embed_bwd_zeroed": (I, [P, P, P, P, P, I, I, I, I, P, P]),
+        "dmi_embed_fwd_ln": (I, [P, P, P, P, L64, I, I, I, P, P, P, P, P, F, P, I, P, P]),
         "dmi_layernorm_fwd": (I, [P, P, P, P, P, P, L64, I, F, P]),
         "dmi_layernorm_bwd_workspace_bytes": (L64, [L64, I]),
         "dmi_layernorm_bwd": (I, [P, P, P, P, P, P, P, P, P, P, L64, I, P]),
@@ -88,6 +91,7 @@
         "dmi_gemm_nt_softmax": (I, [P, I, P, I, P, P, P, I, P, I, I, I, P]),
         "dmi_softmax_finish": (I, [P, I, P, P, P, P, I, P, I, P, P, I, I, P, P, P, P, P, L64, I, I, F, P]),
         "dmi_softmax_finish_w": (I, [P, I, P, P, P, P, I, P, I, P, P, I, I, P, P, P, P, P, L64, I, I, F, P, I, P]),
+        "dmi_softmax_finish_zl": (I, [P, I, P, P, P, I, P, I, P, P, I, I, P, P, P, P, P, L64, I, I, F, P, I, P]),
         "dmi_loss_reduce": (I, [P, L64, P, I, I, F, P, P]),
         "dmi_shift_labels": (I, [P, P, I, I, I, P]),
         "dmi_cross_entropy": (I, [P, I, P, P, P, L64, I, F, P]),
@@ -112,6 +116,7 @@
         "dmi_sumsq_workspace_bytes": (L64, [L64]),
         "dmi_sumsq": (I, [P, L64, P, P, P]),
         "dmi_adam_step": (I, [P, P, P, P, P, L64, P, F, F, F, F, F, F, F, P, P]),
+        "dmi_adam_step_t": (I, [P, P, P, P, P, P, L64, P, I, L64, P, F, F, F, F, F, F, F, P, P]),
         "dmi_adafactor_plan": (I, [P, I, P]),
         "dmi_adafactor_step": (I, [P, I, P, P, P, P, P, P, P, F, F, P, F, F, F, F, P, L64, P]),
         "dmi_cast_f32_bf16": (I, [P, P, L64, P]),
@@ -184,6 +189,12 @@
     _check(lib().dmi_embed_fwd(_p(tokens), _p(wte), _p(wpe), _p(x), tokens.numel(), S, d, vocab, _p(pos_dev), _stream()), "embed_fwd")
 
 
+def embed_fwd_ln(tokens, wte, wpe, x, S, d, vocab, g, b, y, mean, rstd, eps=1e-5, labels=None, eos=0, flag=None):
+    _dev(tokens, wte, wpe, x, g, b, y, mean, rstd, labels, flag)
+    _check(lib().dmi_embed_fwd_ln(_p(tokens), _p(wte), _p(wpe), _p(x), tokens.numel(), S, d, vocab, _p(g), _p(b), _p(y), _p(mean),
+                                  _p(rstd), eps, _p(labels), eos, _p(flag), _stream()), "embed_fwd_ln")
+
+
 def sort_tokens_workspace_bytes(n):
     return int(lib().dmi_sort_tokens_workspace_bytes(n))
 
@@ -201,6 +212,17 @@
     _dev(sorted_tokens, perm, dx, dwte, dwpe, ws)
     _check(lib().dmi_embed_bwd(_p(sorted_tokens), _p(perm), _p(dx), _p(dwte), _p(dwpe), B, S, d, vocab, _p(ws), _stream()),
            "embed_bwd")
+
+
+def embed_bwd_zero(dwte, d, vocab):
+    _dev(dwte)
+    _check(lib().dmi_embed_bwd_zero(_p(dwte), d, vocab, _stream()), "embed_bwd_zero")
+
+
+def embed_bwd_zeroed(sorted_tokens, perm, dx, dwte, dwpe, B, S, d, vocab, ws):
+    _dev(sorted_tokens, perm, dx, dwte, dwpe, ws)
+    _check(lib().dmi_embed_bwd_zeroed(_p(sorted_tokens), _p(perm), _p(dx), _p(dwte), _p(dwpe), B, S, d, vocab, _p(ws), _stream()),
+           "embed_bwd_zeroed")
 
 
 def layernorm_fwd(x, g, b, y, mean, rstd, rows, d, eps=1e-5):
@@ -496,6 +518,14 @@
                                     _p(bias), _p(E), lde, N,
                                     _p(loss_rows), _p(rowscale), _p(rowscale_bf16), _p(Xs), _p(flag), M, K, V, float(dz_scale),
                                     _stream()), "softmax_finish")
+
+
+def softmax_finish_zl(rowsum_part, nparts, label_logit, labels, X, ldx, Wt, ldw, bias, E, lde, N, loss_rows, rowscale,
+                      rowscale_bf16, Xs, flag, M, K, V, dz_scale, pos_weight=None, period=0):
+    _dev(rowsum_part, label_logit, labels, X, Wt, bias, E, loss_rows, flag, pos_weight)
+    _check(lib().dmi_softmax_finish_zl(_p(rowsum_part), nparts, _p(label_logit), _p(labels), _p(X), ldx, _p(Wt), ldw, _p(bias), _p(E),
+                                       lde, N, _p(loss_rows), _p(rowscale), _p(rowscale_bf16), _p(Xs), _p(flag), M, K, V, dz_scale,
+                                       _p(pos_weight), int(period), _stream()), "softmax_finish_zl")
 
 
 def softmax_finish_w(rowsum_part, nparts, label_logit, rowshift, labels, X, ldx, Wt, ldw, bias, E, lde, N, loss_rows, rowscale,
@@ -620,6 +650,13 @@
                                wd, grad_scale, _p(lr_dev), _stream()), "adam_step")
 
 
+def adam_step_t(p, g, m, v, p_bf16, pt_bf16, n, table, ntab, total_tiles, gnorm_sq, clip, lr, beta1, beta2, eps, wd, grad_scale=1.0,
+                lr_dev=None):
+    _dev(p, g, m, v, p_bf16, pt_bf16, table)
+    _check(lib().dmi_adam_step_t(_p(p), _p(g), _p(m), _p(v), _p(p_bf16), _p(pt_bf16), n, _p(table), ntab, total_tiles, _p(gnorm_sq), clip,
+                                 lr, beta1, beta2, eps, wd, grad_scale, _p(lr_dev), _stream()), "adam_step_t")
+
+
 AF_FIELDS = 17
 
 
diff --git a/dalle-mtf_amd/src/dalle_mtf/engine.py b/dalle-mtf_amd/src/dalle_mtf/engine.py
--- a/dalle-mtf_amd/src/dalle_mtf/engine.py
+++ b/dalle-mtf_amd/src/dalle_mtf/engine.py
@@ -314,6 +314,10 @@
     def refresh_compute_copies(self, cast=False):
         if cast:
             dh.cast_f32_bf16(self.p, self.pb, self.lay.total)
+        self._transpose_table()
+        dh.transpose_batch(self.pb, self.pbt, self._t_table, self._t_table.shape[0], self._t_tiles)
+
+    def _transpose_table(self):
         if getattr(self, "_t_table", None) is None:
             rows, tile = [], 0
             for name in self.lay.t_offset:
@@ -322,7 +326,6 @@
                 tile += ((r + 63) // 64) * ((c + 63) // 64)
             self._t_table = torch.tensor(rows, dtype=torch.int64, device=self.dev)
             self._t_tiles = tile
-        dh.transpose_batch(self.pb, self.pbt, self._t_table, self._t_table.shape[0], self._t_tiles)
 
     def _alloc_activations(self):
         M, d, L, B, H, S, Vp = self.M, self.d, self.L, self.B, self.H, self.S, self.Vp
@@ -397,6 +400,9 @@
         self.hp.setdefault("wgrad_group4", os.environ.get("DALLE_WGRAD_GROUP4", "1") != "0")
         self.wgrad_group4 = bool(self.hp["wgrad_group4"] and self.hp["wgrad_pair"] and self.hp["defer_reduces"]
                                  and dh.gemm_tn_group_plan([(4 * d, d), (d, 4 * d), (d, d), (d, 3 * d)], M) > 0)
+        for k in ("adam_transposed", "embed_ln", "finish_label_logit", "early_wte_fill"):
+            self.hp.setdefault(k, os.environ.get("DALLE_" + k.upper(), "1") != "0")
+        self._wte_filled = False
         self.hp.setdefault("lnbwd_chain", os.environ.get("DALLE_LNBWD_CHAIN", "1") != "0")
         self.fuse_lnbwd = bool(self.hp.get("fuse_lnbwd", os.environ.get("DALLE_FUSE_LNBWD", "1") != "0")) and ln_ok
         if self.fuse_lnbwd:
@@ -413,18 +419,29 @@
         assert tokens.shape == (B, S) and tokens.dtype == torch.int32
         self.tokens.copy_(tokens)
         self._sort_done = None
+        self._wte_filled = False
         if need_grad:
             self._launch_sort()
-        dh.shift_labels(self.tokens, self.labels, B, S, self.eos)
-        dh.embed_fwd(self.tokens, self._w("embedding/wte"), self._w("positional_embedding/wpe"), self.X[0], S, d, self.V)
+        fold_zl = need_grad and self.hp["finish_label_logit"]
+        if self.hp["embed_ln"] and L > 0:
+            self._ln1_done = True
+            dh.embed_fwd_ln(self.tokens, self._w("embedding/wte"), self._w("positional_embedding/wpe"), self.X[0], S, d, self.V,
+                            self._w("layer_0/norm_1/g"), self._w("layer_0/norm_1/b"), self.xn1[0], self.stats[0][0], self.stats[0][1],
+                            labels=self.labels, eos=self.eos, flag=self.head_flag)
+        else:
+            dh.shift_labels(self.tokens, self.labels, B, S, self.eos)
+            dh.embed_fwd(self.tokens, self._w("embedding/wte"), self._w("positional_embedding/wpe"), self.X[0], S, d, self.V)
+            if fold_zl:
+                self.head_flag.zero_()
         for l in range(L):
             self._block_forward(l)
+        self._ln1_done = False
         if not (self.fuse_ln1 and L > 0):
             dh.layernorm_fwd(self.X[L], self._w("to_logits/layer_norm/g"), self._w("to_logits/layer_norm/b"), self.xnf,
                              self.statf[0], self.statf[1], M, d)
         Wt, bias = self.tview("to_logits/linear_out/kernel"), self._w("to_logits/linear_out/bias")
         nmb = (self.hp.get("num_microbatches", 1) or 1) if need_grad else 1
-        if need_grad:
+        if need_grad and not fold_zl:
             dh.label_logit(self.xnf, d, Wt, d, bias, self.labels, self.zl, self.head_flag, M, d, self.V)
         hook = getattr(self, "event_hook", None)
         if hook is not None:
@@ -439,7 +456,12 @@
             e1.record()
             hook().append((e0, e1))
         weighted = self.pos_weight is not None
-        if need_grad and weighted:
+        if fold_zl:
+            dh.softmax_finish_zl(self.rowsum_part, self.nparts, self.zl, self.labels, self.xnf, d, Wt, d, bias, self.z, Vp, Vp,
+                                 self.loss_rows, self.rowscale, self.rowscale_bf, self.xs, self.head_flag, M, d, self.V,
+                                 1.0 / (self.B_global * nmb) if weighted else 1.0 / (self.B_global * S * nmb),
+                                 self.pos_weight, S if weighted else 0)
+        elif need_grad and weighted:
             dh.softmax_finish_w(self.rowsum_part, self.nparts, self.zl, None, self.labels, self.xnf, d, Wt, d, bias, self.z, Vp, Vp,
                                 self.loss_rows, self.rowscale, self.rowscale_bf, self.xs, self.head_flag, M, d, self.V,
                                 1.0 / (self.B_global * nmb), self.pos_weight, S)
@@ -461,7 +483,9 @@
         x = self.X[l]
         st = self.stats[l]
         rerun = getattr(self, "_in_backward", False)
-        if not (self.fuse_ln1 and l > 0):
+        if l == 0 and getattr(self, "_ln1_done", False) and not rerun:
+            pass
+        elif not (self.fuse_ln1 and l > 0):
             dh.layernorm_fwd(x, self._w(p + "norm_1/g"), self._w(p + "norm_1/b"), self.xn1[l], st[0], st[1], M, d)
         dh.gemm_nt(self.xn1[l], d, self.tview(p + "attn/qkv"), d, self.qkv[l], 3 * d, M, 3 * d, d)
         self._attn_fwd(l, self.qkv[l], self.o[l], self.lse[l])
@@ -744,6 +768,9 @@
         self.sort_stream.wait_stream(main)
         with torch.cuda.stream(self.sort_stream):
             dh.sort_tokens(self.tokens, self.tok_sorted, self.tok_perm, self.M, self.V, self.sort_ws)
+            self._wte_filled = bool(self.hp["early_wte_fill"])
+            if self._wte_filled:
+                dh.embed_bwd_zero(self._gv("embedding/wte"), self.d, self.V)
             self._sort_done = torch.cuda.Event()
             self._sort_done.record(self.sort_stream)
 
@@ -878,8 +905,9 @@
             ready(rp[1 + bi])
         if self._sort_done is not None:
             torch.cuda.current_stream().wait_event(self._sort_done)
-        dh.embed_bwd(self.tok_sorted, self.tok_perm, dxa, self._gv("embedding/wte"), self._gv("positional_embedding/wpe"),
-                     B, S, d, self.V, self.embed_ws)
+        (dh.embed_bwd_zeroed if self._wte_filled else dh.embed_bwd)(
+            self.tok_sorted, self.tok_perm, dxa, self._gv("embedding/wte"), self._gv("positional_embedding/wpe"), B, S, d, self.V, self.embed_ws)
+        self._wte_filled = False
         flush_ln()
         ready(rp[L + 1])
 
@@ -940,6 +968,12 @@
         if clip is not None:
             dh.sumsq(self.g, n, self.gnorm_sq, self.ws)
             gn, cl = self.gnorm_sq, float(clip)
+        if not wd and self.hp["adam_transposed"]:
+            self._transpose_table()
+            dh.adam_step_t(self.p, self.g, self.m, self.v, self.pb, self.pbt, n, self._t_table, self._t_table.shape[0], self._t_tiles,
+                           gn, cl, lr, b1, b2, eps, 0.0)
+            self.global_step += 1
+            return lr
         if not wd:
             dh.adam_step(self.p, self.g, self.m, self.v, self.pb, n, gn, cl, lr, b1, b2, eps, 0.0)
         else:
diff --git a/include/dalle_hip.h b/include/dalle_hip.h
--- a/include/dalle_hip.h
+++ b/include/dalle_hip.h
@@ -27,6 +27,12 @@
 int64_t dmi_embed_bwd_workspace_bytes(int B, int S, int d);
 int dmi_embed_bwd(const int32_t* sorted_tokens, const int32_t* perm, const uint16_t* dx, float* dwte,
                   float* dwpe, int B, int S, int d, int vocab, void* workspace, void* stream);
+int dmi_embed_bwd_zero(float* dwte, int d, int vocab, void* stream);
+int dmi_embed_bwd_zeroed(const int32_t* sorted_tokens, const int32_t* perm, const uint16_t* dx, float* dwte,
+                         float* dwpe, int B, int S, int d, int vocab, void* workspace, void* stream);
+int dmi_embed_fwd_ln(const int32_t* tokens, const uint16_t* wte, const uint16_t* wpe, uint16_t* x, int64_t rows, int S, int d,
+                     int vocab, const uint16_t* g, const uint16_t* b, uint16_t* y, float* mean, float* rstd, float eps,
+                     int32_t* labels, int eos, int32_t* flag, void* stream);
 
 int dmi_layernorm_fwd(const uint16_t* x, const uint16_t* g, const uint16_t* b, uint16_t* y,
                       float* mean, float* rstd, int64_t rows, int d, float eps, void* stream);
@@ -120,6 +126,10 @@
                        const uint16_t* Wt, int ldw, const uint16_t* bias, uint16_t* E, int lde, int N,
                        float* loss_rows, float* rowscale, uint16_t* rowscale_bf16, uint16_t* Xs, int32_t* flag,
                        int64_t M, int K, int V, float dz_scale, void* stream);
+int dmi_softmax_finish_zl(const float* rowsum_part, int nparts, float* label_logit, const int32_t* labels,
+                          const uint16_t* X, int ldx, const uint16_t* Wt, int ldw, const uint16_t* bias, uint16_t* E, int lde,
+                          int N, float* loss_rows, float* rowscale, uint16_t* rowscale_bf16, uint16_t* Xs, int32_t* flag,
+                          int64_t M, int K, int V, float dz_scale, const float* pos_weight, int period, void* stream);
 int dmi_sum_f32(const float* x, int64_t n, float scale, float* out, void* stream);
 int dmi_softmax_finish_w(const float* rowsum_part, int nparts, const float* label_logit, const float* rowshift,
                          const int32_t* labels, const uint16_t* X, int ldx,
@@ -152,6 +162,9 @@
 int dmi_adam_step(float* p, const float* g, float* m, float* v, uint16_t* p_bf16, int64_t n,
                   const float* gnorm_sq, float clip, float lr, float beta1, float beta2, float eps,
                   float weight_decay, float grad_scale, const float* lr_dev, void* stream);
+int dmi_adam_step_t(float* p, const float* g, float* m, float* v, uint16_t* p_bf16, uint16_t* pt_bf16, int64_t n,
+                    const int64_t* table, int ntab, int64_t total_tiles, const float* gnorm_sq, float clip, float lr, float beta1,
+                    float beta2, float eps, float weight_decay, float grad_scale, const float* lr_dev, void* stream);
 
 #define DMI_AF_FIELDS 17
 int dmi_adafactor_plan(int64_t* table, int nvars, int64_t* totals);
```

Result: no change. 2.824 million (median of 4 runs) (+0.0%).
